# SkylerGao/MC_NeRF

Measured on AMD Instinct MI355X. Metric: train rays/sec (coarse+fine, 64+128 samples), higher is better.
Workload: dtype f16x3h; 1 GPU; Ball_Lego-shaped 110-view 800x800, coarse 4x128 @64 + fine 8x256 @128-grid, GLOBAL_OPTIM stage, fwd+bwd+allreduce+RAdam; precision=f16x3h, parallelism=dp1

## Files before the change

### mc_nerf_amd/build.py

```python
import os
import subprocess
import sys
from concurrent.futures import ThreadPoolExecutor

HERE = os.path.dirname(os.path.abspath(__file__))
CSRC = os.path.join(HERE, "csrc")
OUT = os.path.join(HERE, "libmcnerf.so")
SOURCES = ["api.hip", "pack.hip", "mlp_fwd.hip", "mlp_bwd.hip", "mlp_dw.hip", "pack16.hip", "mlp16_fwd.hip", "mlp16_bwd.hip", "mlp16_dw.hip", "mlp_x3_fwd.hip", "mlp_x3_bwd.hip", "mlp_x3_dw.hip", "composite.hip", "sample_pdf.hip", "select.hip", "rays.hip", "voxel.hip", "optim.hip", "optim_rows.hip", "camera.hip", "color_calib.hip", "errmap.hip", "lens.hip"]
HEADERS = ["mcnerf_common.h", "mcnerf_kernels.h", "mcnerf_wave.h", "mcnerf_16.h", "mcnerf_x3.h", "mcnerf_launch.h", "mcnerf_voxel.h", "mcnerf_multicam.h", "mcnerf_colorcal.h", "mcnerf_errmap.h", "mcnerf_maxkey.h", "mcnerf_compact.h", "mcnerf_hash.h", "mcnerf_rays.h", "mcnerf_lens.h", "mcnerf_optim_rows.h", os.path.join("..", "..", "include", "mcnerf.h")]
FILE_FLAGS = {s: ["-mllvm", "-pragma-unroll-threshold=200000", "-mllvm", "-amdgpu-mfma-vgpr-form"] for s in ("mlp_x3_fwd.hip", "mlp_x3_bwd.hip")}
FLAGS = ["--offload-arch=gfx950", "-O3", "-std=c++17", "-fPIC", "-munsafe-fp-atomics", "-ffp-contract=off", "-fno-slp-vectorize", "-Wall", "-Wno-unused-function"]


def _newer(a, b):
    return (not os.path.exists(b)) or os.path.getmtime(a) > os.path.getmtime(b)


def build(force=False, verbose=True):
    hipcc = os.environ.get("HIPCC", "/opt/rocm/bin/hipcc")
    objdir = os.path.join(HERE, "build")
    os.makedirs(objdir, exist_ok=True)
    hdrs = [os.path.normpath(os.path.join(CSRC, h)) for h in HEADERS]
    jobs = []
    for s in SOURCES:
        src, obj = os.path.join(CSRC, s), os.path.join(objdir, s.replace(".hip", ".o"))
        if force or _newer(src, obj) or any(_newer(h, obj) for h in hdrs):
            jobs.append((src, obj))

    def cc(job):
        src, obj = job
        cmd = [hipcc] + FLAGS + FILE_FLAGS.get(os.path.basename(src), []) + ["-c", src, "-o", obj]
        r = subprocess.run(cmd, capture_output=True, text=True)
        return src, r.returncode, r.stdout + r.stderr

    with ThreadPoolExecutor(max_workers=min(4, max(1, len(jobs)))) as ex:
        for src, rc, log in ex.map(cc, jobs):
            if verbose and log.strip():
                print(log)
            if rc != 0:
                raise RuntimeError(f"hipcc failed on {src}\n{log}")
            if verbose:
                print(f"[mc_nerf_amd.build] compiled {os.path.basename(src)}")
    objs = [os.path.join(objdir, s.replace(".hip", ".o")) for s in SOURCES]
    if jobs or not os.path.exists(OUT):
        cmd = [hipcc, "--offload-arch=gfx950", "-shared", "-fPIC", "-o", OUT] + objs
        r = subprocess.run(cmd, capture_output=True, text=True)
        if r.returncode != 0:
            raise RuntimeError("link failed\n" + r.stdout + r.stderr)
        if verbose:
            print(f"[mc_nerf_amd.build] linked {OUT}")
    return OUT


if __name__ == "__main__":
    build(force="--force" in sys.argv)
```

### mc_nerf_amd/csrc/mcnerf_x3.h

```cpp
#pragma once
#include "mcnerf_16.h"

#define MCNX3_SW 256.0f
#define MCNX3_SX 8.0f
#define MCNX3_SLABF 8
#define MCNX3_PF 2

#define MCNX3_WIDE_MIN 128
static inline constexpr int mcnx3_waves(int width) { return width >= MCNX3_WIDE_MIN ? 4 : 8; }

static inline int mcnx3_pad(int frags) { return (frags + MCNX3_SLABF - 1) / MCNX3_SLABF * MCNX3_SLABF; }
static inline Mcn16Stream mcnx3_repad(Mcn16Stream st) {
    int total = 0;
    for (int s = 0; s < st.nseg; ++s) {
        st.seg[s].first_frag = total;
        total += mcnx3_pad(st.seg[s].tiles * (st.seg[s].a.ksteps + st.seg[s].b.ksteps));
    }
    st.total_frags = total;
    return st;
}
static inline Mcn16Stream mcnx3_fwd_stream(const McnLayout& L) { return mcnx3_repad(mcn16_fwd_stream(L)); }
static inline Mcn16Stream mcnx3_bwd_stream(const McnLayout& L) { return mcnx3_repad(mcn16_bwd_stream(L)); }

static inline size_t mcnx3_slot_bytes(long long capacity, int width) { return 2 * mcn16_slot_bytes(capacity, width); }
static inline size_t mcnx3_enc_bytes(long long capacity) { return 2 * mcn16_enc_bytes(capacity); }
static inline size_t mcnx3_sh_bytes(long long capacity) { return (size_t)mcn16_cap_tiles(capacity) * 4096; }
static inline size_t mcnx3_dsh_bytes(long long capacity) { return 2 * mcn16_dsh_bytes(capacity); }

hipError_t mcnx3_launch_fwd(const Mcn16FwdArgs& a, hipStream_t st);
hipError_t mcnx3_launch_bwd(const Mcn16BwdArgs& a, hipStream_t st);
hipError_t mcnx3_launch_dw(const Mcn16DwArgs& a, hipStream_t st);
hipError_t mcnx3_launch_pack(const McnLayout& L, const float* params, void* packed_fwd, void* packed_bwd, unsigned* range_flags, hipStream_t st);

#ifdef __HIPCC__
typedef float f32x2_t __attribute__((ext_vector_type(2)));

__device__ __forceinline__ void mcnx3_split2(float a, float b, unsigned& hi, unsigned& lo) {
    const f16x2_t h = __builtin_convertvector((f32x2_t){a, b}, f16x2_t);
    const f32x2_t back = __builtin_convertvector(h, f32x2_t);
    const f16x2_t l = __builtin_convertvector((f32x2_t){a - back[0], b - back[1]}, f16x2_t);
    hi = __builtin_bit_cast(unsigned, h);
    lo = __builtin_bit_cast(unsigned, l);
}
__device__ __forceinline__ float mcnx3_val(unsigned hi, unsigned lo, int e) {
    const f16x2_t h = __builtin_bit_cast(f16x2_t, hi), l = __builtin_bit_cast(f16x2_t, lo);
    return (float)h[e] + (float)l[e];
}
template <int HI>
__device__ __forceinline__ float mcnx3_residual(float v, unsigned hw) {
    float r;
    if (HI) asm("v_fma_mix_f32 %0, %1, -1.0, %2 op_sel:[1,0,0] op_sel_hi:[1,0,0]" : "=v"(r) : "v"(hw), "v"(v));
    else asm("v_fma_mix_f32 %0, %1, -1.0, %2 op_sel_hi:[1,0,0]" : "=v"(r) : "v"(hw), "v"(v));
    return r;
}
__device__ __forceinline__ float mcnx3_relu(float x) {
    const int i = __builtin_bit_cast(int, x);
    return __builtin_bit_cast(float, i > 0 ? i : 0);
}
__device__ __forceinline__ f32x16 mcnx3_mfma(const u32x4_t& a, const u32x4_t& b, const f32x16& c) {
    return __builtin_amdgcn_mfma_f32_32x32x16_f16(__builtin_bit_cast(f16x8_t, a), __builtin_bit_cast(f16x8_t, b), c, 0, 0, 0);
}
__device__ __forceinline__ void mcnx3_mfma3(f32x16& acc, const u32x4_t& ah, const u32x4_t& al, const u32x4_t& bh, const u32x4_t& bl) {
    acc = mcnx3_mfma(al, bh, acc);
    acc = mcnx3_mfma(ah, bl, acc);
    acc = mcnx3_mfma(ah, bh, acc);
}

__device__ __forceinline__ void mcnx3_dma16(const char* ubase, unsigned voff, unsigned lds_dst) {
    unsigned keep;
    asm volatile("s_mov_b32 %0, m0\n\ts_mov_b32 m0, %3\n\ts_nop 0\n\tglobal_load_lds_dwordx4 %1, %2\n\ts_mov_b32 m0, %0"
                 : "=&s"(keep) : "v"(voff), "s"(ubase), "s"(lds_dst) : "memory");
}
template <int PPW>
__device__ __forceinline__ void mcnx3_ring_issue(Mcn16Ring& r) {
    const char* s = r.ubase + (size_t)r.src_slab * (MCN16_SLAB * 1024);
    const unsigned d = r.lds_base + r.issue_slot * (MCN16_SLAB * 1024) + r.lds_piece;
#pragma unroll
    for (int i = 0; i < PPW; ++i) mcnx3_dma16(s + i * 1024, r.voff, d + i * 1024);
    r.src_slab = (r.src_slab + 1 == r.n_slabs) ? 0 : r.src_slab + 1;
    r.issue_slot = (r.issue_slot + 1) & (MCN16_RING - 1);
}
template <int PPW>
__device__ __forceinline__ void mcnx3_ring_sync(Mcn16Ring& r) {
    asm volatile("s_waitcnt vmcnt(%0)\n\ts_barrier" ::"n"(PPW * (MCN16_AHEAD - 1)) : "memory");
    r.next_off = r.sync_slot * (MCN16_SLAB * 1024);
    r.sync_slot = (r.sync_slot + 1) & (MCN16_RING - 1);
    mcnx3_ring_issue<PPW>(r);
}
template <int PPW>
__device__ __forceinline__ void mcnx3_ring_start(Mcn16Ring& r, char* ring_lds, const void* packed, int n_slabs, int wave, int lane) {
    r.ubase = reinterpret_cast<const char*>(packed) + (PPW * wave) * 1024;
    r.voff = lane * 16;
    r.src = nullptr;
    r.lds_piece = (PPW * wave) * 1024;
    r.lds_base = (unsigned)reinterpret_cast<size_t>((mcn16_lds_ptr_t)ring_lds);
    r.src_slab = 0; r.n_slabs = n_slabs; r.issue_slot = 0; r.sync_slot = 0; r.next_off = 0;
#pragma unroll
    for (int i = 0; i < MCN16_AHEAD; ++i) mcnx3_ring_issue<PPW>(r);
    mcnx3_ring_sync<PPW>(r);
}
template <int F>
__host__ __device__ constexpr int mcnx3_sync_at(int q) {
    return (MCNX3_SLABF * q + MCNX3_SLABF - MCNX3_PF) < (F - 1) ? (MCNX3_SLABF * q + MCNX3_SLABF - MCNX3_PF) : (F - 1);
}
template <int F, int PPW>
__device__ __forceinline__ void mcnx3_before_mfma(Mcn16Ring& r, Mcn16Cursor& c, int f) {
    if ((f & (MCNX3_SLABF - 1)) == 0) c.cur = r.next_off;
    if (f == mcnx3_sync_at<F>(f / MCNX3_SLABF)) mcnx3_ring_sync<PPW>(r);
}
#define MCNX3_DMA_STEP 2
template <int PPW>
__device__ __forceinline__ void mcnx3_ring_piece(Mcn16Ring& r, int i) {
    switch (i) {
        case 0: asm volatile("global_load_lds_dwordx4 %0, %1" ::"v"(r.voff), "s"(r.piece_base) : "memory"); break;
        case 1: asm volatile("global_load_lds_dwordx4 %0, %1 offset:1024" ::"v"(r.voff), "s"(r.piece_base) : "memory"); break;
        case 2: asm volatile("global_load_lds_dwordx4 %0, %1 offset:2048" ::"v"(r.voff), "s"(r.piece_base) : "memory"); break;
        default: asm volatile("global_load_lds_dwordx4 %0, %1 offset:3072" ::"v"(r.voff), "s"(r.piece_base) : "memory"); break;
    }
}
template <int F, int PPW>
__device__ __forceinline__ void mcnx3_before_mfma_spread(Mcn16Ring& r, Mcn16Cursor& c, int f) {
    static_assert(PPW <= 4, "immediate offsets of the refill pieces");
    if ((f & (MCNX3_SLABF - 1)) == 0) c.cur = r.next_off;
    if (f == mcnx3_sync_at<F>(f / MCNX3_SLABF)) {
        asm volatile("s_waitcnt vmcnt(%0)\n\ts_barrier" ::"n"(PPW * (MCN16_AHEAD - 1)) : "memory");
        r.next_off = r.sync_slot * (MCN16_SLAB * 1024);
        r.sync_slot = (r.sync_slot + 1) & (MCN16_RING - 1);
        r.piece_base = r.ubase + (size_t)r.src_slab * (MCN16_SLAB * 1024);
        asm volatile("s_mov_b32 m0, %0" ::"s"(r.lds_base + r.issue_slot * (MCN16_SLAB * 1024) + r.lds_piece) : "memory");
        r.src_slab = (r.src_slab + 1 == r.n_slabs) ? 0 : r.src_slab + 1;
        r.issue_slot = (r.issue_slot + 1) & (MCN16_RING - 1);
    }
}
template <int F, int PPW>
__device__ __forceinline__ void mcnx3_gap_dma(Mcn16Ring& r, int gap) {
    constexpr int NQ = (F + MCNX3_SLABF - 1) / MCNX3_SLABF;
#pragma unroll
    for (int q = 0; q < NQ; ++q)
#pragma unroll
        for (int i = 0; i < PPW; ++i)
            if (gap == 3 * mcnx3_sync_at<F>(q) + 1 + MCNX3_DMA_STEP * i) mcnx3_ring_piece<PPW>(r, i);
}
template <int F, int PPW>
__device__ __forceinline__ void mcnx3_layer_end(Mcn16Ring& r) {
    constexpr int NQ = (F + MCNX3_SLABF - 1) / MCNX3_SLABF;
#pragma unroll
    for (int q = 0; q < NQ; ++q)
#pragma unroll
        for (int i = 0; i < PPW; ++i)
            if (3 * mcnx3_sync_at<F>(q) + 1 + MCNX3_DMA_STEP * i >= 3 * F) mcnx3_ring_piece<PPW>(r, i);
}
__device__ __forceinline__ unsigned mcnx3_frag_off(const Mcn16Ring& r, const Mcn16Cursor& c, int f_now, int f) {
    const bool next = (f / MCNX3_SLABF) != (f_now / MCNX3_SLABF);
    return (next ? r.next_off : c.cur) + (f & (MCNX3_SLABF - 1)) * 2048;
}

__device__ __forceinline__ void mcnx3_encode_values(const float (&p)[3], const float (&bw)[MCN_NFREQ], float (&E)[64]) {
    E[0] = p[0]; E[1] = p[1]; E[2] = p[2]; E[63] = 0.f;
#pragma unroll
    for (int a = 0; a < 3; ++a) {
        float S[MCN_NFREQ], C[MCN_NFREQ];
        mcn_sincos_octaves<MCN_NFREQ>(p[a], S, C);
#pragma unroll
        for (int f = 0; f < MCN_NFREQ; ++f) {
            E[3 + 20 * a + f] = S[f] * bw[f];
            E[3 + 20 * a + 10 + f] = C[f] * bw[f];
        }
    }
}
#endif
```

### mc_nerf_amd/csrc/mlp_x3_bwd.hip

```cpp
#include "mcnerf_x3.h"
#include "mcnerf_launch.h"

#define MCNX3_BWD_PREF_MINW 256
#include <cstdlib>

template <int W>
struct BwdX3Smem {
    static constexpr int WAVES = mcnx3_waves(W);
    static constexpr int oW2 = MCN16_RING * MCN16_SLAB * 1024;
    static constexpr int oBarf = oW2 + W * 4;
    static constexpr int MW = W >= 64 ? W / 64 : 1;
    static constexpr int oMask = oBarf + 16 * 4;
    static constexpr int oIdx = oMask + WAVES * 3 * MW * 256;
    static constexpr int oIn = oIdx + WAVES * 256;
    static constexpr int total = oIn + (W >= 256 ? WAVES * 16 * 256 : 0);
};

template <int W, int KSTEPS, int NTILES, int MODE, int PPW, bool HI>
__device__ __forceinline__ void mcnx3_bwd_seg(Mcn16Ring& ring, char* smem, int lane,
                                              const u32x4_t (&inh)[W / 16], const u32x4_t (&inl)[W / 16],
                                              u32x4_t (&outh)[W / 16], u32x4_t (&outl)[W / 16],
                                              const unsigned (&mk)[W >= 64 ? W / 64 : 1], f32x16 (&acc2)[2], char* save_lane) {
    constexpr int KS = W / 16, F = NTILES * KSTEPS, G = 3 * KSTEPS;
    constexpr bool EPI = MODE != 3;
    constexpr int NIT = EPI ? (MODE == 0 ? 16 : 20) : 0;
    constexpr int START = (G >= NIT + 8) ? 3 : 0;
    constexpr int IPG = EPI ? (NIT + (G - START) - 1) / (G - START) : 1;
    constexpr int LASTA = EPI ? START + 14 / IPG : 0;
    constexpr int SBASE = START + 16, SSTR = (G - SBASE) / 4 > 0 ? (G - SBASE) / 4 : 1;
    constexpr bool STAG = (MODE == 1 || MODE == 2) && IPG == 1 && (G - SBASE) / 4 >= 2;
    constexpr int NITG = STAG ? 16 : NIT;
    constexpr int INIT_G = (G - 8) > LASTA ? (G - 8) : LASTA;
    constexpr int INIT_N = (INIT_G + 3 <= G - 1) ? 4 : 1;
    Mcn16Cursor cur;
    u32x4_t afh[MCNX3_PF], afl[MCNX3_PF];
    f32x16 acc[2];
    float v0 = 0.f, v1 = 0.f;
    unsigned wkeep = 0u;
    auto acc_init = [&](f32x16& a, int t, int q) {
        if (MODE == 2) {
            const f16x8_t h8 = __builtin_bit_cast(f16x8_t, outh[2 * t + (q >> 1)]), l8 = __builtin_bit_cast(f16x8_t, outl[2 * t + (q >> 1)]);
#pragma unroll
            for (int e = 0; e < 4; ++e) a[4 * q + e] = ((float)h8[4 * (q & 1) + e] + (float)l8[4 * (q & 1) + e]) * MCNX3_SW;
        } else {
#pragma unroll
            for (int e = 0; e < 4; ++e) a[4 * q + e] = 0.f;
        }
    };
    auto item = [&](const f32x16& a, int t, int i) {
        if (i < 16) {
            const int p = i >> 1;
            const unsigned bits = MODE != 0 ? ((mk[t >> 1] >> (8 * (t & 1) + 7 - p)) & 0x00010001u) : 0u;
            if ((i & 1) == 0) {
                v0 = a[2 * p] * (1.0f / MCNX3_SW);
                v1 = a[2 * p + 1] * (1.0f / MCNX3_SW);
                const unsigned w = Mcn16T<false>::pack(v0, v1);
                wkeep = w;
                outh[2 * t + (p >> 2)][p & 3] = MODE != 0 ? mcn16_pkmul(w, bits) : w;
            } else {
                const unsigned w = Mcn16T<false>::pack(mcnx3_residual<0>(v0, wkeep), mcnx3_residual<1>(v1, wkeep));
                outl[2 * t + (p >> 2)][p & 3] = MODE != 0 ? mcn16_pkmul(w, bits) : w;
            }
        } else {
            const int k = i - 16, s = 2 * t + (k & 1);
            if (k < 2) mcn16_ws_store(outh[s], reinterpret_cast<u32x4_t*>(save_lane + s * 1024));
            else if (!HI) mcn16_ws_store(outl[s], reinterpret_cast<u32x4_t*>(save_lane + (KS + s) * 1024));
        }
    };
    cur.cur = ring.next_off;
#pragma unroll
    for (int i = 0; i < MCNX3_PF; ++i)
        if (i < F) {
            afh[i] = *reinterpret_cast<const u32x4_t*>(smem + ring.next_off + i * 2048 + lane * 16);
            afl[i] = *reinterpret_cast<const u32x4_t*>(smem + ring.next_off + i * 2048 + 1024 + lane * 16);
        }
    if (EPI) {
#pragma unroll
        for (int q = 0; q < 4; ++q) acc_init(acc[0], 0, q);
    }
#pragma unroll
    for (int t = 0; t < NTILES; ++t) {
#pragma unroll
        for (int s = 0; s < KSTEPS; ++s) {
            const int f = t * KSTEPS + s;
            mcnx3_before_mfma_spread<F, PPW>(ring, cur, f);
            const u32x4_t a_h = afh[f % MCNX3_PF], a_l = afl[f % MCNX3_PF];
            if (f + MCNX3_PF < F) {
                const unsigned o = mcnx3_frag_off(ring, cur, f, f + MCNX3_PF) + lane * 16;
                afh[f % MCNX3_PF] = *reinterpret_cast<const u32x4_t*>(smem + o);
                afl[f % MCNX3_PF] = *reinterpret_cast<const u32x4_t*>(smem + o + 1024);
            }
#pragma unroll
            for (int g = 0; g < 3; ++g) {
                const int gap = 3 * s + g;
                if (EPI && t > 0 && gap >= START) {
#pragma unroll
                    for (int i = (gap - START) * IPG; i < (gap - START + 1) * IPG; ++i)
                        if (i < NITG) item(acc[(t - 1) & 1], t - 1, i);
                    if (STAG && gap >= SBASE && (gap - SBASE) / SSTR < 4 && (gap - SBASE) % SSTR == 0)
                        item(acc[(t - 1) & 1], t - 1, 16 + (gap - SBASE) / SSTR);
                }
                if (EPI && t + 1 < NTILES && gap >= INIT_G && gap < INIT_G + INIT_N) {
#pragma unroll
                    for (int q = 0; q < 4; ++q)
                        if (INIT_N == 1 || q == gap - INIT_G) acc_init(acc[(t + 1) & 1], t + 1, q);
                }
                mcnx3_gap_dma<F, PPW>(ring, 3 * f + g);
                __builtin_amdgcn_sched_barrier(0);
                if (EPI) acc[t & 1] = mcnx3_mfma(g == 0 ? a_l : a_h, g == 1 ? inl[s] : inh[s], acc[t & 1]);
                else acc2[t & 1] = mcnx3_mfma(g == 0 ? a_l : a_h, g == 1 ? inl[s] : inh[s], acc2[t & 1]);
                __builtin_amdgcn_sched_barrier(0);
            }
        }
    }
    mcnx3_layer_end<F, PPW>(ring);
    if (EPI) {
#pragma unroll
        for (int i = 0; i < NIT; ++i) item(acc[(NTILES - 1) & 1], NTILES - 1, i);
    }
}

template <int W, bool HI>
__global__ __launch_bounds__(64 * mcnx3_waves(W), mcnx3_waves(W) / 4) void mlp_x3_bwd_kernel(Mcn16BwdArgs a) {
    using SM = BwdX3Smem<W>;
    constexpr int PL = HI ? 1 : 2;
    constexpr int WAVES = mcnx3_waves(W), ROWS = 32 * WAVES, PPW = 16 / WAVES;
    constexpr int NT = W / 32, KS = W / 16, MW = W >= 64 ? W / 64 : 1;
    extern __shared__ __attribute__((aligned(16))) char smem[];
    const int tid = threadIdx.x, lane = tid & 63, wave = __builtin_amdgcn_readfirstlane(tid >> 6);
    const int m = lane & 31, h = lane >> 5;
    const int D = a.lay.depth, skip = a.lay.skip;
    const long long total = a.count ? (long long)min(*a.count, a.max_rows) : (long long)a.n_rays * a.S;
    if ((long long)blockIdx.x * ROWS >= total) return;

    float* sw2 = reinterpret_cast<float*>(smem + SM::oW2);
    for (int i = tid; i < W; i += 64 * WAVES) sw2[i] = a.params[a.lay.pWs2 + i];
    float* sbarf = reinterpret_cast<float*>(smem + SM::oBarf);
    if (tid < MCN_NFREQ) sbarf[tid] = a.barf_w[tid];
    const float gmax = __uint_as_float(*a.gmax_bits);
    const float sg = mcn16_grad_scale(gmax);
    const float inv_sg = 1.0f / sg;
    __syncthreads();

    struct In { int ray; float zg, jit; f32x4 o, go; float dx, dy, dz, ox, oy, oz; };
    auto gather = [&](int ray, int j) -> In {
        In r;
        r.ray = ray;
        r.zg = a.zgrid[ray * a.z_stride + j];
        r.jit = a.jitter ? a.jitter[ray] : 0.f;
        const size_t addr = (size_t)ray * a.S + j;
        r.o = *reinterpret_cast<const f32x4*>(a.out + addr * 4);
        r.go = *reinterpret_cast<const f32x4*>(a.d_out + addr * 4);
        r.dx = a.rays_d[ray * 3]; r.dy = a.rays_d[ray * 3 + 1]; r.dz = a.rays_d[ray * 3 + 2];
        r.ox = a.rays_o[ray * 3]; r.oy = a.rays_o[ray * 3 + 1]; r.oz = a.rays_o[ray * 3 + 2];
        return r;
    };
    auto row_of = [&](long long pass_) -> long long {
        const long long g_ = (pass_ * WAVES + wave) * 32 + m;
        return g_ < total ? g_ : total - 1;
    };
    constexpr bool PREFB = W >= MCNX3_BWD_PREF_MINW;
    constexpr int SLABS_FULL = (W / 32) * (W / 16) / MCNX3_SLABF;
    constexpr int SLABS_ENC = (2 * (W / 16) + MCNX3_SLABF - 1) / MCNX3_SLABF;
    constexpr int N_IDX = PPW * (2 * SLABS_FULL - 1) < 63 ? PPW * (2 * SLABS_FULL - 1) : 63;
    constexpr int N_TOP = PPW * (SLABS_FULL + SLABS_ENC - 1) < 63 ? PPW * (SLABS_FULL + SLABS_ENC - 1) : 63;
    const unsigned in_lds = (unsigned)reinterpret_cast<size_t>((mcn16_lds_ptr_t)smem) + SM::oIn + wave * (16 * 256);
    const float* in_rd = reinterpret_cast<const float*>(smem + SM::oIn + wave * (16 * 256)) + lane;
    auto gather_dma = [&](int ray, int j) {
        mcn16_dma4(a.zgrid + ray * a.z_stride + j, in_lds);
        if (a.jitter) mcn16_dma4(a.jitter + ray, in_lds + 256);
        const size_t addr = ((size_t)ray * a.S + j) * 4;
#pragma unroll
        for (int c = 0; c < 4; ++c) {
            mcn16_dma4(a.out + addr + c, in_lds + (2 + c) * 256);
            mcn16_dma4(a.d_out + addr + c, in_lds + (6 + c) * 256);
        }
#pragma unroll
        for (int c = 0; c < 3; ++c) {
            mcn16_dma4(a.rays_d + ray * 3 + c, in_lds + (10 + c) * 256);
            mcn16_dma4(a.rays_o + ray * 3 + c, in_lds + (13 + c) * 256);
        }
    };
    auto read_in = [&](int ray) -> In {
        In r;
        r.ray = ray;
        r.zg = in_rd[0];
        r.jit = a.jitter ? in_rd[64] : 0.f;
        r.o = f32x4{in_rd[2 * 64], in_rd[3 * 64], in_rd[4 * 64], in_rd[5 * 64]};
        r.go = f32x4{in_rd[6 * 64], in_rd[7 * 64], in_rd[8 * 64], in_rd[9 * 64]};
        r.dx = in_rd[10 * 64]; r.dy = in_rd[11 * 64]; r.dz = in_rd[12 * 64];
        r.ox = in_rd[13 * 64]; r.oy = in_rd[14 * 64]; r.oz = in_rd[15 * 64];
        return r;
    };
    In cur;
    int ray_n = 0;
    {
        const long long gc0 = row_of(blockIdx.x);
        int ray0, j0;
        if (a.idx) { const int2 rj = a.idx[gc0]; ray0 = rj.x; j0 = rj.y; }
        else { ray0 = (int)(gc0 / a.S); j0 = (int)(gc0 - (long long)ray0 * a.S); }
        if (PREFB) { gather_dma(ray0, j0); ray_n = ray0; }
        else cur = gather(ray0, j0);
    }

    Mcn16Ring ring;
    mcnx3_ring_start<PPW>(ring, smem, a.packed, a.stream_slabs, wave, lane);
    const float* w2_h = sw2 + 4 * h;
    const unsigned idx_lds = (unsigned)reinterpret_cast<size_t>((mcn16_lds_ptr_t)smem) + SM::oIdx + wave * 256;

    constexpr bool MASK_DMA = W >= MCNX3_BWD_PREF_MINW;
    const unsigned mlds = ring.lds_base + SM::oMask + wave * (3 * MW * 256);
    auto mask_issue = [&](const unsigned* mask_lane, int slot, int buf) {
        if (MASK_DMA) {
#pragma unroll
            for (int i = 0; i < MW; ++i) mcn16_dma4(mask_lane + (size_t)slot * a.mask_slot_words + i, mlds + (buf * MW + i) * 256);
        }
    };
    auto mask_read = [&](const unsigned* mask_lane, unsigned (&mk)[MW], int buf, int slot) {
#pragma unroll
        for (int i = 0; i < MW; ++i) {
            if (MASK_DMA) mk[i] = *reinterpret_cast<const unsigned*>(smem + SM::oMask + wave * (3 * MW * 256) + (buf * MW + i) * 256 + lane * 4);
            else mk[i] = mask_lane[(size_t)slot * a.mask_slot_words + i];
        }
    };
    auto buf_of = [&](int slot) { return (D + 1 - slot) % 3; };
    auto mask_lane_of = [&](long long pass_) { return a.mask_ws + ((size_t)(pass_ * WAVES + wave) * 64 + lane) * MW; };
    unsigned mk0_s[MW], mk0_c[MW], mk0_t[MW];
    {
        const unsigned* ml0 = mask_lane_of(blockIdx.x);
        mask_issue(ml0, D, 0); mask_issue(ml0, D + 1, 1); mask_issue(ml0, D - 1, 2);
        if (!MASK_DMA) { mask_read(ml0, mk0_s, 0, D); mask_read(ml0, mk0_c, 1, D + 1); mask_read(ml0, mk0_t, 2, D - 1); }
        asm volatile("s_waitcnt vmcnt(0)" ::: "memory");
    }

    for (long long pass = blockIdx.x; pass * ROWS < total; pass += gridDim.x) {
        const long long tile = pass * WAVES + wave;
        const long long g = tile * 32 + m;
        const bool valid = g < total;
        const unsigned* mask_lane = mask_lane_of(pass);
        char* dy_lane = reinterpret_cast<char*>(a.dy_ws) + (size_t)tile * (PL * KS) * 1024 + lane * 16;
        if (PREFB) {
            asm volatile("s_waitcnt vmcnt(%0)" ::"n"(N_TOP) : "memory");
            cur = read_in(ray_n);
        }
        const int ray = cur.ray;
        unsigned mk_s[MW], mk_c[MW], mk_t[MW];
        float zv = cur.zg;
        if (a.jitter) zv = __fadd_rn(zv, cur.jit);
        const f32x4 o = cur.o;
        f32x4 go = cur.go;
        if (!valid) go = f32x4{0.f, 0.f, 0.f, 0.f};
        const float x = cur.dx, y = cur.dy, z = cur.dz;
        float p[3];
        p[0] = __fadd_rn(cur.ox, __fmul_rn(x, zv));
        p[1] = __fadd_rn(cur.oy, __fmul_rn(y, zv));
        p[2] = __fadd_rn(cur.oz, __fmul_rn(z, zv));
        float bas[9];
        mcn_sh_basis(x, y, z, bas);
        float dpre[3];
#pragma unroll
        for (int c = 0; c < 3; ++c) dpre[c] = go[1 + c] * o[1 + c] * (1.f - o[1 + c]) * sg;
        const float dsg = go[0] * sg;
        u32x4_t dshh[2], dshl[2];
#pragma unroll
        for (int s = 0; s < 2; ++s)
#pragma unroll
            for (int d = 0; d < 4; ++d) {
                float v[2];
#pragma unroll
                for (int u = 0; u < 2; ++u) {
                    const int n0 = mcn16_chan(s, 0, 2 * d + u), n1 = n0 + 4;
                    const float va = n0 < MCN_NSH ? dpre[n0 / 9] * bas[n0 % 9] : (n0 == MCN_NSH ? dsg : 0.f);
                    const float vb = n1 < MCN_NSH ? dpre[n1 / 9] * bas[n1 % 9] : (n1 == MCN_NSH ? dsg : 0.f);
                    v[u] = h ? vb : va;
                }
                unsigned wh, wl;
                mcnx3_split2(v[0], v[1], wh, wl);
                dshh[s][d] = wh; dshl[s][d] = wl;
            }
        {
            char* e = reinterpret_cast<char*>(a.dsh_ws) + (size_t)tile * (PL * 2) * 1024 + lane * 16;
            mcn16_ws_store(dshh[0], reinterpret_cast<u32x4_t*>(e));
            mcn16_ws_store(dshh[1], reinterpret_cast<u32x4_t*>(e + 1024));
            if (!HI) {
                mcn16_ws_store(dshl[0], reinterpret_cast<u32x4_t*>(e + 2048));
                mcn16_ws_store(dshl[1], reinterpret_cast<u32x4_t*>(e + 3072));
            }
        }

        if (MASK_DMA) mask_read(mask_lane, mk_s, 0, D);
        else {
#pragma unroll
            for (int i = 0; i < MW; ++i) { mk_s[i] = mk0_s[i]; mk_c[i] = mk0_c[i]; mk_t[i] = mk0_t[i]; }
        }
        const long long pass_n = pass + gridDim.x;
        if (a.idx) {
            const long long gn = (pass_n * WAVES + wave) * 32 + (lane >> 1);
            mcn16_dma4(reinterpret_cast<const int*>(a.idx) + 2 * (gn < total ? gn : total - 1) + (lane & 1), idx_lds);
        }
        const bool want_rays = a.d_rays_o || a.d_rays_d;
        f32x4 shs[4];
#pragma unroll
        for (int q = 0; q < 4; ++q) shs[q] = f32x4{0.f, 0.f, 0.f, 0.f};
        if (PREFB && want_rays) {
#pragma unroll
            for (int q = 0; q < 4; ++q)
                shs[q] = *reinterpret_cast<const f32x4*>(reinterpret_cast<const char*>(a.sh_ws) + (size_t)tile * 4096 + q * 1024 + lane * 16);
        }
        u32x4_t xah[KS], xal[KS], xbh[KS], xbl[KS];
        f32x16 denc[2];
#pragma unroll
        for (int t = 0; t < 2; ++t)
#pragma unroll
            for (int e = 0; e < 16; ++e) denc[t][e] = 0.f;
#pragma unroll
        for (int s = 0; s < KS; ++s) {
            const f32x4 wa = *reinterpret_cast<const f32x4*>(w2_h + 16 * s), wb = *reinterpret_cast<const f32x4*>(w2_h + 16 * s + 8);
            const int t = s >> 1;
#pragma unroll
            for (int d = 0; d < 4; ++d) {
                const float va = (d < 2 ? wa[2 * d] : wb[2 * d - 4]) * dsg, vb = (d < 2 ? wa[2 * d + 1] : wb[2 * d - 3]) * dsg;
                const int i = 4 * (s & 1) + d;
                const unsigned bits = (mk_s[t >> 1] >> (8 * (t & 1) + 7 - i)) & 0x00010001u;
                unsigned wh, wl;
                mcnx3_split2(va, vb, wh, wl);
                xah[s][d] = mcn16_pkmul(wh, bits);
                xal[s][d] = mcn16_pkmul(wl, bits);
            }
            mcn16_ws_store(xah[s], reinterpret_cast<u32x4_t*>(dy_lane + (size_t)D * a.slot_bytes + s * 1024));
            if (!HI) mcn16_ws_store(xal[s], reinterpret_cast<u32x4_t*>(dy_lane + (size_t)D * a.slot_bytes + (KS + s) * 1024));
        }
        if (D >= 2) mask_issue(mask_lane, D - 2, buf_of(D - 2));
        unsigned mpend[MW];
        if (!MASK_DMA && D >= 2) mask_read(mask_lane, mpend, 0, D - 2);
        mcnx3_bwd_seg<W, KS, NT, 0, PPW, HI>(ring, smem, lane, xah, xal, xbh, xbl, mk_s, denc, nullptr);
        if (MASK_DMA) mask_read(mask_lane, mk_c, 1, D + 1);
        {
            u32x4_t dih[KS], dil[KS];
            dih[0] = dshh[0]; dih[1] = dshh[1]; dil[0] = dshl[0]; dil[1] = dshl[1];
            mcnx3_bwd_seg<W, 2, NT, 1, PPW, HI>(ring, smem, lane, dih, dil, xah, xal, mk_c, denc, dy_lane + (size_t)(D + 1) * a.slot_bytes);
        }
        if (D >= 3) mask_issue(mask_lane, D - 3, buf_of(D - 3));
        if (MASK_DMA) mask_read(mask_lane, mk_t, 2, D - 1);
        mcnx3_bwd_seg<W, KS, NT, 2, PPW, HI>(ring, smem, lane, xah, xal, xbh, xbl, mk_t, denc, dy_lane + (size_t)(D - 1) * a.slot_bytes);
        auto trunk_masks = [&](int l) {
            if (MASK_DMA) {
                if (l >= 3) mask_issue(mask_lane, l - 3, buf_of(l - 3));
                mask_read(mask_lane, mk_t, buf_of(l - 1), l - 1);
            } else {
#pragma unroll
                for (int i = 0; i < MW; ++i) mk_t[i] = mpend[i];
                if (l >= 2) mask_read(mask_lane, mpend, 0, l - 2);
            }
            if (l == 1 && pass_n * ROWS < total) {
                const unsigned* mln = mask_lane_of(pass_n);
                mask_issue(mln, D, 0); mask_issue(mln, D + 1, 1); mask_issue(mln, D - 1, 2);
                if (!MASK_DMA) { mask_read(mln, mk0_s, 0, D); mask_read(mln, mk0_c, 1, D + 1); mask_read(mln, mk0_t, 2, D - 1); }
            }
        };
        auto next_rows = [&]() {
            asm volatile("s_waitcnt vmcnt(%0)" ::"n"(N_IDX) : "memory");
            int rn, jn;
            if (a.idx) {
                const int2 rj = *reinterpret_cast<const int2*>(smem + SM::oIdx + wave * 256 + m * 8);
                rn = rj.x; jn = rj.y;
            } else {
                const long long gn = row_of(pass_n);
                rn = (int)(gn / a.S); jn = (int)(gn - (long long)rn * a.S);
            }
            gather_dma(rn, jn);
            ray_n = rn;
        };
        for (int l = D - 1; l >= 1; l -= 2) {
            if (PREFB && l == 1) next_rows();
            trunk_masks(l);
            if (l == skip) mcnx3_bwd_seg<W, KS, 2, 3, PPW, HI>(ring, smem, lane, xbh, xbl, xah, xal, mk_t, denc, nullptr);
            mcnx3_bwd_seg<W, KS, NT, 1, PPW, HI>(ring, smem, lane, xbh, xbl, xah, xal, mk_t, denc, dy_lane + (size_t)(l - 1) * a.slot_bytes);
            if (l - 1 >= 1) {
                if (PREFB && l - 1 == 1) next_rows();
                trunk_masks(l - 1);
                if (l - 1 == skip) mcnx3_bwd_seg<W, KS, 2, 3, PPW, HI>(ring, smem, lane, xah, xal, xbh, xbl, mk_t, denc, nullptr);
                mcnx3_bwd_seg<W, KS, NT, 1, PPW, HI>(ring, smem, lane, xah, xal, xbh, xbl, mk_t, denc, dy_lane + (size_t)(l - 2) * a.slot_bytes);
            } else {
#pragma unroll
                for (int s = 0; s < KS; ++s) { xbh[s] = xah[s]; xbl[s] = xal[s]; }
            }
        }
        In nxt = cur;
        if (PREFB && D < 2) {
            next_rows();
        }
        if (!PREFB) {
            int rn, jn;
            if (a.idx) {
                const int2 rj = *reinterpret_cast<const int2*>(smem + SM::oIdx + wave * 256 + m * 8);
                rn = rj.x; jn = rj.y;
            } else {
                const long long gn = row_of(pass_n);
                rn = (int)(gn / a.S); jn = (int)(gn - (long long)rn * a.S);
            }
            nxt = gather(rn, jn);
        }
        if (!PREFB && want_rays) {
#pragma unroll
            for (int q = 0; q < 4; ++q)
                shs[q] = *reinterpret_cast<const f32x4*>(reinterpret_cast<const char*>(a.sh_ws) + (size_t)tile * 4096 + q * 1024 + lane * 16);
        }
        mcnx3_bwd_seg<W, KS, 2, 3, PPW, HI>(ring, smem, lane, xbh, xbl, xah, xal, mk_t, denc, nullptr);
        auto settle = [&]() {
            if (PREFB && D >= 2) return;
            asm volatile("s_waitcnt vmcnt(0)" ::: "memory");
            asm volatile("" : "+v"(nxt.ray), "+v"(nxt.zg), "+v"(nxt.jit), "+v"(nxt.o), "+v"(nxt.go));
            asm volatile("" : "+v"(nxt.dx), "+v"(nxt.dy), "+v"(nxt.dz), "+v"(nxt.ox), "+v"(nxt.oy), "+v"(nxt.oz));
            if (!MASK_DMA) {
#pragma unroll
                for (int i = 0; i < MW; ++i) asm volatile("" : "+v"(mk0_s[i]), "+v"(mk0_c[i]), "+v"(mk0_t[i]));
            }
        };

        if (want_rays) {
            auto dch = [&](int ch) -> float {
                const int hh = (ch >> 2) & 1;
                const float v = denc[ch >> 5][4 * ((ch >> 3) & 3) + (ch & 3)];
                return (h == hh) ? v : 0.f;
            };
            float dpos[3];
#pragma unroll
            for (int ax = 0; ax < 3; ++ax) {
                float acc = dch(ax);
                float S[MCN_NFREQ], C[MCN_NFREQ];
                mcn_sincos_octaves<MCN_NFREQ>(p[ax], S, C);
#pragma unroll
                for (int f = 0; f < MCN_NFREQ; ++f) {
                    const float k = (float)(1 << f) * sbarf[f];
                    acc = fmaf(k * C[f], dch(3 + 20 * ax + f), acc);
                    acc = fmaf(-k * S[f], dch(3 + 20 * ax + 10 + f), acc);
                }
                dpos[ax] = acc * (1.0f / MCNX3_SW);
            }
            float ddir[3] = {0.f, 0.f, 0.f};
            {
                const float C1 = 0.4886025119029199f, C20 = 1.0925484305920792f, C22 = 0.31539156525252005f, C24 = 0.5462742152960396f;
                const float gx[9] = {0.f, 0.f, 0.f, -C1, C20 * y, 0.f, -2.f * C22 * x, -C20 * z, 2.f * C24 * x};
                const float gy[9] = {0.f, -C1, 0.f, 0.f, C20 * x, -C20 * z, -2.f * C22 * y, 0.f, -2.f * C24 * y};
                const float gz[9] = {0.f, 0.f, C1, 0.f, 0.f, -C20 * y, 4.f * C22 * z, -C20 * x, 0.f};
#pragma unroll
                for (int r = 0; r < 16; ++r) {
                    const float v = shs[r >> 2][r & 3];
                    const int n0 = 8 * (r >> 2) + (r & 3), n1 = n0 + 4;
                    const float kx = h ? (n1 < MCN_NSH ? dpre[n1 / 9] * gx[n1 % 9] : 0.f) : (n0 < MCN_NSH ? dpre[n0 / 9] * gx[n0 % 9] : 0.f);
                    const float ky = h ? (n1 < MCN_NSH ? dpre[n1 / 9] * gy[n1 % 9] : 0.f) : (n0 < MCN_NSH ? dpre[n0 / 9] * gy[n0 % 9] : 0.f);
                    const float kz = h ? (n1 < MCN_NSH ? dpre[n1 / 9] * gz[n1 % 9] : 0.f) : (n0 < MCN_NSH ? dpre[n0 / 9] * gz[n0 % 9] : 0.f);
                    ddir[0] = fmaf(kx, v, ddir[0]); ddir[1] = fmaf(ky, v, ddir[1]); ddir[2] = fmaf(kz, v, ddir[2]);
                }
            }
            float red[6];
#pragma unroll
            for (int c = 0; c < 3; ++c) {
                const float dp = dpos[c] + __shfl_xor(dpos[c], 32);
                const float dd = ddir[c] + __shfl_xor(ddir[c], 32);
                red[c] = dp * inv_sg;
                red[3 + c] = (dp * zv + dd) * inv_sg;
            }
            settle();
            const int rkey = valid ? ray : -1;
            const int rprev = __shfl_up(rkey, 1, 32);
            int head = (m == 0 || rprev != rkey) ? 1 : 0;
#pragma unroll
            for (int off = 1; off < 32; off <<= 1) {
                const int hup = __shfl_up(head, off, 32);
                const bool take = (m >= off) && !head;
#pragma unroll
                for (int c = 0; c < 6; ++c) {
                    const float up = __shfl_up(red[c], off, 32);
                    red[c] += take ? up : 0.f;
                }
                if (m >= off) head |= hup;
            }
            const int rnext = __shfl_down(rkey, 1, 32);
            if (h == 0 && valid && (m == 31 || rnext != rkey)) {
#pragma unroll
                for (int c = 0; c < 3; ++c) {
                    if (a.d_rays_o) atomicAdd(a.d_rays_o + ray * 3 + c, red[c]);
                    if (a.d_rays_d) atomicAdd(a.d_rays_d + ray * 3 + c, red[3 + c]);
                }
            }
        }
        if (!want_rays) settle();
        if (!PREFB) cur = nxt;
    }
    asm volatile("s_waitcnt vmcnt(0)" ::: "memory");
}

hipError_t mcnx3_launch_bwd(const Mcn16BwdArgs& a, hipStream_t st) {
    return mcn_for_width(a.lay.width, [&](auto w) {
        constexpr int W = decltype(w)::value, WAVES = mcnx3_waves(W);
        void (*kern)(Mcn16BwdArgs) = mcn16_hi_planes_only(a.dtype) ? mlp_x3_bwd_kernel<W, true> : mlp_x3_bwd_kernel<W, false>;
        return mcn_launch(kern, mcn_persistent_grid(mcn_passes(mcn_max_rows(a), 32 * WAVES)), 64 * WAVES, BwdX3Smem<W>::total, st, a);
    });
}
```

### mc_nerf_amd/csrc/mlp_x3_fwd.hip

```cpp
#include "mcnerf_x3.h"
#include "mcnerf_launch.h"

template <int W>
struct FwdX3Smem {
    static constexpr int oBias = MCN16_RING * MCN16_SLAB * 1024;
    static constexpr int oW2 = oBias + (MCN_MAXD + 2) * W * 4;
    static constexpr int oBc2 = oW2 + W * 4;
    static constexpr int oIdx = oBc2 + 32 * 4;
    static constexpr int oIn = oIdx + mcnx3_waves(W) * 256;
    static constexpr int total = oIn + mcnx3_waves(W) * 8 * 256;
};

template <int W, int SV, int KENC, int KHID, int EPI, int PPW>
__device__ __forceinline__ void mcnx3_layer(Mcn16Ring& ring, char* smem, int lane,
                                            const u32x4_t (&ench)[MCN16_ENCKS], const u32x4_t (&encl)[MCN16_ENCKS],
                                            const u32x4_t (&inh)[W / 16], const u32x4_t (&inl)[W / 16],
                                            u32x4_t (&outh)[W / 16], u32x4_t (&outl)[W / 16], const float* bias_h,
                                            const float* w2_h, float& dot, char* save_lane, unsigned* mask_lane) {
    constexpr bool SAVE = SV != 0, HI = SV == 2;
    constexpr int NT = W / 32, KS = W / 16, KTOT = KENC + KHID, F = NT * KTOT, MW = W >= 64 ? W / 64 : 1;
    constexpr int G = 3 * KTOT;
    constexpr bool HAS2 = SAVE || EPI == 1;
    constexpr int IPW = HAS2 ? 3 : 2;
    constexpr int NST = SAVE ? (HI ? 2 : 4) : 0;
    constexpr int NIT = 8 * IPW + NST;
    constexpr int NWI = 8 * IPW;
    constexpr int ROOM = G - 3 - 2 * NST;
    constexpr int IPGA = ROOM > 0 ? (NWI + ROOM - 1) / ROOM : 99;
    constexpr bool STAG = SAVE && IPGA <= 2;
    constexpr int START = STAG ? 3 : (G >= NIT + 4 ? 3 : 0);
    constexpr int IPG = STAG ? IPGA : (NIT + (G - START) - 1) / (G - START);
    constexpr int NITG = STAG ? NWI : NIT;
    constexpr int LASTG = START + (NITG + IPG - 1) / IPG - 1;
    constexpr int SBASE = LASTG + 1, SSTR = STAG ? (G - SBASE) / NST : 1;
    constexpr int BIAS_G = (G - 6) > LASTG ? (G - 6) : LASTG;
    Mcn16Cursor cur;
    unsigned mw[MW];
#pragma unroll
    for (int i = 0; i < MW; ++i) mw[i] = 0u;
    u32x4_t afh[MCNX3_PF], afl[MCNX3_PF];
    f32x16 acc[2];
    unsigned mb = 0u;
    float v0 = 0.f, v1 = 0.f;
    unsigned wkeep = 0u;
    auto bias_init = [&](f32x16& a, int t) {
#pragma unroll
        for (int q = 0; q < 4; ++q) {
            const f32x4 b = *reinterpret_cast<const f32x4*>(bias_h + 32 * t + 8 * q);
#pragma unroll
            for (int e = 0; e < 4; ++e) a[4 * q + e] = b[e];
        }
    };
    auto item = [&](const f32x16& a, int t, int i) {
        if (i < 8 * IPW) {
            const int p = i / IPW, ph = i % IPW;
            if (ph == 0) {
                v0 = mcnx3_relu(a[2 * p] * (1.0f / MCNX3_SW));
                v1 = mcnx3_relu(a[2 * p + 1] * (1.0f / MCNX3_SW));
                const unsigned w = Mcn16T<false>::pack(v0, v1);
                wkeep = w;
                outh[2 * t + (p >> 2)][p & 3] = w;
            } else if (ph == IPW - 1) {
                outl[2 * t + (p >> 2)][p & 3] = Mcn16T<false>::pack(mcnx3_residual<0>(v0, wkeep), mcnx3_residual<1>(v1, wkeep));
            } else {
                if (SAVE) {
                    mb = (p == 0) ? mcn16_nz(wkeep) : ((mb << 1) | mcn16_nz(wkeep));
                    if (p == 7) mw[t >> 1] |= mb << (8 * (t & 1));
                }
                if (EPI == 1) {
                    const f32x2_t ww = *reinterpret_cast<const f32x2_t*>(w2_h + 32 * t + 8 * (p >> 1) + 2 * (p & 1));
                    dot = fmaf(v0, ww[0], dot);
                    dot = fmaf(v1, ww[1], dot);
                }
            }
        } else if (SAVE) {
            const int k = i - 8 * IPW;
            const int s = 2 * t + (k & 1);
            if (k < 2) mcn16_ws_store(outh[s], reinterpret_cast<u32x4_t*>(save_lane + s * 1024));
            else mcn16_ws_store(outl[s], reinterpret_cast<u32x4_t*>(save_lane + (KS + s) * 1024));
        }
    };
    cur.cur = ring.next_off;
#pragma unroll
    for (int i = 0; i < MCNX3_PF; ++i)
        if (i < F) {
            afh[i] = *reinterpret_cast<const u32x4_t*>(smem + ring.next_off + i * 2048 + lane * 16);
            afl[i] = *reinterpret_cast<const u32x4_t*>(smem + ring.next_off + i * 2048 + 1024 + lane * 16);
        }
    bias_init(acc[0], 0);
#pragma unroll
    for (int t = 0; t < NT; ++t) {
#pragma unroll
        for (int s = 0; s < KTOT; ++s) {
            const int f = t * KTOT + s;
            mcnx3_before_mfma_spread<F, PPW>(ring, cur, f);
            const u32x4_t a_h = afh[f % MCNX3_PF], a_l = afl[f % MCNX3_PF];
            if (f + MCNX3_PF < F) {
                const unsigned o = mcnx3_frag_off(ring, cur, f, f + MCNX3_PF) + lane * 16;
                afh[f % MCNX3_PF] = *reinterpret_cast<const u32x4_t*>(smem + o);
                afl[f % MCNX3_PF] = *reinterpret_cast<const u32x4_t*>(smem + o + 1024);
            }
            const u32x4_t b_h = s < KENC ? ench[s < KENC ? s : 0] : inh[s >= KENC ? s - KENC : 0];
            const u32x4_t b_l = s < KENC ? encl[s < KENC ? s : 0] : inl[s >= KENC ? s - KENC : 0];
#pragma unroll
            for (int g = 0; g < 3; ++g) {
                const int gap = 3 * s + g;
                if (t > 0 && gap >= START) {
#pragma unroll
                    for (int i = (gap - START) * IPG; i < (gap - START + 1) * IPG; ++i)
                        if (i < NITG) item(acc[(t - 1) & 1], t - 1, i);
                    if (STAG && gap >= SBASE && (gap - SBASE) / SSTR < NST && (gap - SBASE) % SSTR == 0)
                        item(acc[(t - 1) & 1], t - 1, 8 * IPW + (gap - SBASE) / SSTR);
                }
                if (gap == BIAS_G && t + 1 < NT) bias_init(acc[(t + 1) & 1], t + 1);
                mcnx3_gap_dma<F, PPW>(ring, 3 * f + g);
                __builtin_amdgcn_sched_barrier(0);
                acc[t & 1] = mcnx3_mfma(g == 0 ? a_l : a_h, g == 1 ? b_l : b_h, acc[t & 1]);
                __builtin_amdgcn_sched_barrier(0);
            }
        }
    }
    mcnx3_layer_end<F, PPW>(ring);
#pragma unroll
    for (int i = 0; i < NIT; ++i) item(acc[(NT - 1) & 1], NT - 1, i);
    if (SAVE) {
#pragma unroll
        for (int i = 0; i < MW; ++i) mcn16_ws_store(mw[i], mask_lane + i);
    }
}


template <int W, int SV>
__global__ __launch_bounds__(64 * mcnx3_waves(W), mcnx3_waves(W) / 4) void mlp_x3_fwd_kernel(Mcn16FwdArgs a) {
    using SM = FwdX3Smem<W>;
    constexpr bool SAVE = SV != 0, HI = SV == 2;
    constexpr int PL = HI ? 1 : 2;
    constexpr int WAVES = mcnx3_waves(W), ROWS = 32 * WAVES, PPW = 16 / WAVES;
    constexpr int KS = W / 16, MW = W >= 64 ? W / 64 : 1;
    constexpr float SXW = MCNX3_SX * MCNX3_SW;
    extern __shared__ __attribute__((aligned(16))) char smem[];
    const int tid = threadIdx.x, lane = tid & 63, wave = __builtin_amdgcn_readfirstlane(tid >> 6);
    const int m = lane & 31, h = lane >> 5;
    const int D = a.lay.depth, skip = a.lay.skip;
    const long long total = a.count ? (long long)min(*a.count, a.max_rows) : (long long)a.n_rays * a.S;
    if ((long long)blockIdx.x * ROWS >= total) return;

    float* sbias = reinterpret_cast<float*>(smem + SM::oBias);
    float* sw2 = reinterpret_cast<float*>(smem + SM::oW2);
    float* sbc2 = reinterpret_cast<float*>(smem + SM::oBc2);
    for (int l = 0; l < D; ++l)
        for (int i = tid; i < W; i += 64 * WAVES) sbias[l * W + i] = a.params[a.lay.pB[l] + i] * SXW;
    for (int i = tid; i < W; i += 64 * WAVES) {
        sbias[D * W + i] = a.params[a.lay.pBs1 + i] * SXW;
        sbias[(D + 1) * W + i] = a.params[a.lay.pBc1 + i] * SXW;
        sw2[i] = a.params[a.lay.pWs2 + i];
    }
    if (tid < 32) {
        const int row = tid < MCN_NSH ? mcn_sh_row(tid, a.lay.sh_deg) : -1;
        sbc2[tid] = row >= 0 ? a.params[a.lay.pBc2 + row] * SXW : 0.f;
    }
    const float bs2 = a.params[a.lay.pBs2];
    float bw[MCN_NFREQ];
#pragma unroll
    for (int f = 0; f < MCN_NFREQ; ++f) bw[f] = a.barf_w[f];
    __syncthreads();

    constexpr bool PREF = WAVES == 4;
    constexpr int SLABS_FULL = (W / 32) * (W / 16) / MCNX3_SLABF, SLABS_L0 = ((W / 32) * MCN16_ENCKS + MCNX3_SLABF - 1) / MCNX3_SLABF;
    constexpr int SLABS_SH2 = (W / 16 + MCNX3_SLABF - 1) / MCNX3_SLABF;
    constexpr int N_IDX = PPW * (SLABS_L0 + SLABS_FULL - 1) < 63 ? PPW * (SLABS_L0 + SLABS_FULL - 1) : 63;
    constexpr int N_TOP = PPW * (SLABS_FULL + SLABS_SH2 - 1) < 63 ? PPW * (SLABS_FULL + SLABS_SH2 - 1) : 63;
    const unsigned idx_lds = (unsigned)reinterpret_cast<size_t>((mcn16_lds_ptr_t)smem) + SM::oIdx + wave * 256;
    const unsigned in_lds = (unsigned)reinterpret_cast<size_t>((mcn16_lds_ptr_t)smem) + SM::oIn + wave * (8 * 256);
    const float* in_rd = reinterpret_cast<const float*>(smem + SM::oIn + wave * (8 * 256)) + lane;
    auto row_of = [&](long long pass_) -> long long {
        const long long g_ = (pass_ * WAVES + wave) * 32 + m;
        return g_ < total ? g_ : total - 1;
    };
    auto gather_dma = [&](int ray_, int j_) {
        mcn16_dma4(a.zgrid + ray_ * a.z_stride + j_, in_lds);
        if (a.jitter) mcn16_dma4(a.jitter + ray_, in_lds + 256);
#pragma unroll
        for (int c = 0; c < 3; ++c) {
            mcn16_dma4(a.rays_d + ray_ * 3 + c, in_lds + (2 + c) * 256);
            mcn16_dma4(a.rays_o + ray_ * 3 + c, in_lds + (5 + c) * 256);
        }
    };
    int ray_n = 0, j_n = 0;
    {
        const long long gc0 = row_of(blockIdx.x);
        if (a.idx) { const int2 rj = a.idx[gc0]; ray_n = rj.x; j_n = rj.y; }
        else { ray_n = (int)(gc0 / a.S); j_n = (int)(gc0 - (long long)ray_n * a.S); }
        if (PREF) {
            gather_dma(ray_n, j_n);
            asm volatile("s_waitcnt vmcnt(0)" ::: "memory");
        }
    }

    Mcn16Ring ring;
    mcnx3_ring_start<PPW>(ring, smem, a.packed, a.stream_slabs, wave, lane);

    const float* bias_h = sbias + 4 * h;
    const float* w2_h = sw2 + 4 * h;

    for (long long pass = blockIdx.x; pass * ROWS < total; pass += gridDim.x) {
        const long long tile = pass * WAVES + wave;
        const long long g = tile * 32 + m;
        const bool valid = g < total;
        const long long gc = valid ? g : total - 1;
        const long long pass_n = pass + gridDim.x;
        int ray, j;
        float zv, dx, dy, dz, ox, oy, oz;
        if (PREF) {
            ray = ray_n; j = j_n;
            asm volatile("s_waitcnt vmcnt(%0)" ::"n"(N_TOP) : "memory");
            zv = in_rd[0];
            if (a.jitter) zv = __fadd_rn(zv, in_rd[64]);
            dx = in_rd[2 * 64]; dy = in_rd[3 * 64]; dz = in_rd[4 * 64];
            ox = in_rd[5 * 64]; oy = in_rd[6 * 64]; oz = in_rd[7 * 64];
        } else {
            if (a.idx) { const int2 rj = a.idx[gc]; ray = rj.x; j = rj.y; }
            else { ray = (int)(gc / a.S); j = (int)(gc - (long long)ray * a.S); }
            zv = a.zgrid[ray * a.z_stride + j];
            if (a.jitter) zv = __fadd_rn(zv, a.jitter[ray]);
            dx = a.rays_d[ray * 3 + 0]; dy = a.rays_d[ray * 3 + 1]; dz = a.rays_d[ray * 3 + 2];
            ox = a.rays_o[ray * 3 + 0]; oy = a.rays_o[ray * 3 + 1]; oz = a.rays_o[ray * 3 + 2];
        }
        float p[3];
        p[0] = __fadd_rn(ox, __fmul_rn(dx, zv));
        p[1] = __fadd_rn(oy, __fmul_rn(dy, zv));
        p[2] = __fadd_rn(oz, __fmul_rn(dz, zv));
        if (PREF && a.idx) {
            const long long gn = (pass_n * WAVES + wave) * 32 + (lane >> 1);
            mcn16_dma4(reinterpret_cast<const int*>(a.idx) + 2 * (gn < total ? gn : total - 1) + (lane & 1), idx_lds);
        }
        const int addr = ray * a.S + j;
        u32x4_t ench[MCN16_ENCKS], encl[MCN16_ENCKS];
        {
            float E[64];
            mcnx3_encode_values(p, bw, E);
#pragma unroll
            for (int s = 0; s < MCN16_ENCKS; ++s)
#pragma unroll
                for (int d = 0; d < 4; ++d) {
                    const int c0 = mcn16_chan(s, 0, 2 * d), c1 = mcn16_chan(s, 0, 2 * d + 1);
                    unsigned wh, wl;
                    mcnx3_split2((h ? E[c0 + 4] : E[c0]) * MCNX3_SX, (h ? E[c1 + 4] : E[c1]) * MCNX3_SX, wh, wl);
                    ench[s][d] = wh; encl[s][d] = wl;
                }
        }
        char* act_lane = SAVE ? reinterpret_cast<char*>(a.act_ws) + (size_t)tile * (PL * KS) * 1024 + lane * 16 : nullptr;
        unsigned* mask_lane = SAVE ? a.mask_ws + ((size_t)tile * 64 + lane) * MW : nullptr;
        if (SAVE) {
            char* e = reinterpret_cast<char*>(a.enc_ws) + (size_t)tile * (PL * MCN16_ENCKS) * 1024 + lane * 16;
#pragma unroll
            for (int s = 0; s < MCN16_ENCKS; ++s) {
                mcn16_ws_store(ench[s], reinterpret_cast<u32x4_t*>(e + s * 1024));
                if (!HI) mcn16_ws_store(encl[s], reinterpret_cast<u32x4_t*>(e + (MCN16_ENCKS + s) * 1024));
            }
        }

        u32x4_t xah[KS], xal[KS], xbh[KS], xbl[KS];
        float dot = 0.f;
        mcnx3_layer<W, SV, MCN16_ENCKS, 0, 0, PPW>(ring, smem, lane, ench, encl, xah, xal, xbh, xbl, bias_h, nullptr, dot, act_lane, mask_lane);
        for (int l = 1; l < D; l += 2) {
            char* sl = SAVE ? act_lane + (size_t)l * a.slot_bytes : nullptr;
            unsigned* ml = SAVE ? mask_lane + (size_t)l * a.mask_slot_words : nullptr;
            if (l == skip) mcnx3_layer<W, SV, MCN16_ENCKS, KS, 0, PPW>(ring, smem, lane, ench, encl, xbh, xbl, xah, xal, bias_h + l * W, nullptr, dot, sl, ml);
            else mcnx3_layer<W, SV, 0, KS, 0, PPW>(ring, smem, lane, ench, encl, xbh, xbl, xah, xal, bias_h + l * W, nullptr, dot, sl, ml);
            if (l + 1 < D) {
                sl = SAVE ? act_lane + (size_t)(l + 1) * a.slot_bytes : nullptr;
                ml = SAVE ? mask_lane + (size_t)(l + 1) * a.mask_slot_words : nullptr;
                if (l + 1 == skip) mcnx3_layer<W, SV, MCN16_ENCKS, KS, 0, PPW>(ring, smem, lane, ench, encl, xah, xal, xbh, xbl, bias_h + (l + 1) * W, nullptr, dot, sl, ml);
                else mcnx3_layer<W, SV, 0, KS, 0, PPW>(ring, smem, lane, ench, encl, xah, xal, xbh, xbl, bias_h + (l + 1) * W, nullptr, dot, sl, ml);
            } else {
#pragma unroll
                for (int s = 0; s < KS; ++s) { xbh[s] = xah[s]; xbl[s] = xal[s]; }
            }
        }
        mcnx3_layer<W, SV, 0, KS, 1, PPW>(ring, smem, lane, ench, encl, xbh, xbl, xah, xal, bias_h + D * W, w2_h, dot,
                                            SAVE ? act_lane + (size_t)D * a.slot_bytes : nullptr, SAVE ? mask_lane + (size_t)D * a.mask_slot_words : nullptr);
        if (PREF) {
            asm volatile("s_waitcnt vmcnt(%0)" ::"n"(N_IDX) : "memory");
            if (a.idx) {
                const int2 rj = *reinterpret_cast<const int2*>(smem + SM::oIdx + wave * 256 + m * 8);
                ray_n = rj.x; j_n = rj.y;
            } else {
                const long long gn = row_of(pass_n);
                ray_n = (int)(gn / a.S); j_n = (int)(gn - (long long)ray_n * a.S);
            }
            gather_dma(ray_n, j_n);
        }
        mcnx3_layer<W, SV, 0, KS, 0, PPW>(ring, smem, lane, ench, encl, xbh, xbl, xah, xal, bias_h + (D + 1) * W, nullptr, dot,
                                            SAVE ? act_lane + (size_t)(D + 1) * a.slot_bytes : nullptr, SAVE ? mask_lane + (size_t)(D + 1) * a.mask_slot_words : nullptr);
        f32x16 acc;
#pragma unroll
        for (int q = 0; q < 4; ++q) {
            const f32x4 b = *reinterpret_cast<const f32x4*>(sbc2 + 8 * q + 4 * h);
#pragma unroll
            for (int e = 0; e < 4; ++e) acc[4 * q + e] = b[e];
        }
        {
            Mcn16Cursor cur;
#pragma unroll
            for (int s = 0; s < KS; ++s) {
                mcnx3_before_mfma<KS, PPW>(ring, cur, s);
                const unsigned o = cur.cur + (s & (MCNX3_SLABF - 1)) * 2048 + lane * 16;
                const u32x4_t a_h = *reinterpret_cast<const u32x4_t*>(smem + o);
                const u32x4_t a_l = *reinterpret_cast<const u32x4_t*>(smem + o + 1024);
                mcnx3_mfma3(acc, a_h, a_l, xah[s], xal[s]);
            }
        }
#pragma unroll
        for (int e = 0; e < 16; ++e) acc[e] *= 1.0f / SXW;
        if (SAVE) {
            char* e = reinterpret_cast<char*>(a.sh_ws) + (size_t)tile * 4096 + lane * 16;
#pragma unroll
            for (int q = 0; q < 4; ++q)
                mcn16_ws_store(f32x4{acc[4 * q], acc[4 * q + 1], acc[4 * q + 2], acc[4 * q + 3]}, reinterpret_cast<f32x4*>(e + q * 1024));
        }
        float bas[9];
        mcn_sh_basis(dx, dy, dz, bas);
        float pre[3] = {0.f, 0.f, 0.f};
#pragma unroll
        for (int r = 0; r < 16; ++r) {
            const int n0 = 8 * (r >> 2) + (r & 3), n1 = n0 + 4;
            const float b0 = n0 < MCN_NSH ? bas[n0 % 9] : 0.f, b1 = n1 < MCN_NSH ? bas[n1 % 9] : 0.f;
            const float contrib = acc[r] * (h ? b1 : b0);
            const int c0 = n0 / 9, c1 = n1 / 9;
#pragma unroll
            for (int c = 0; c < 3; ++c) {
                const bool in0 = n0 < MCN_NSH && c0 == c, in1 = n1 < MCN_NSH && c1 == c;
                if (in0 && in1) pre[c] += contrib;
                else if (in0) pre[c] += h ? 0.f : contrib;
                else if (in1) pre[c] += h ? contrib : 0.f;
            }
        }
        const float sigma = (dot + __shfl_xor(dot, 32)) * (1.0f / MCNX3_SX) + bs2;
        f32x4 o;
        o[0] = sigma;
#pragma unroll
        for (int c = 0; c < 3; ++c) {
            const float pc = pre[c] + __shfl_xor(pre[c], 32);
            o[1 + c] = 1.0f / (1.0f + expf(-pc));
        }
        if (valid && h == 0) *reinterpret_cast<f32x4*>(a.out + (size_t)addr * 4) = o;
    }
    asm volatile("s_waitcnt vmcnt(0)" ::: "memory");
}

hipError_t mcnx3_launch_fwd(const Mcn16FwdArgs& a, hipStream_t st) {
    return mcn_for_width(a.lay.width, [&](auto w) {
        constexpr int W = decltype(w)::value, WAVES = mcnx3_waves(W);
        void (*kern)(Mcn16FwdArgs) = !a.act_ws ? mlp_x3_fwd_kernel<W, 0> : mcn16_hi_planes_only(a.dtype) ? mlp_x3_fwd_kernel<W, 2> : mlp_x3_fwd_kernel<W, 1>;
        return mcn_launch(kern, mcn_persistent_grid(mcn_passes(mcn_max_rows(a), 32 * WAVES)), 64 * WAVES, FwdX3Smem<W>::total, st, a);
    });
}
```

Baseline: 1.092 million rays/s.

## Add 8-wave variant of x3 MLP fwd/bwd kernels for width 128

Adds an alternate kernel instantiation for width-128 x3 MLP forward and backward that uses 8 waves per block instead of 4. It uses prefetch depth 1, drops the LDS mask staging and reloads lane-dependent addresses through an opaque value to keep register pressure low. Tail tiles are remapped so duplicate 'twin' tiles redo the last live work. The intent is more waves in flight to hide LDS and MFMA latency. The cost is extra address recomputation and shuffles via ds_bpermute, and an environment override can pick the wave count.

```diff
diff --git a/mc_nerf_amd/build.py b/mc_nerf_amd/build.py
--- a/mc_nerf_amd/build.py
+++ b/mc_nerf_amd/build.py
@@ -7,7 +7,7 @@
 CSRC = os.path.join(HERE, "csrc")
 OUT = os.path.join(HERE, "libmcnerf.so")
 SOURCES = ["api.hip", "pack.hip", "mlp_fwd.hip", "mlp_bwd.hip", "mlp_dw.hip", "pack16.hip", "mlp16_fwd.hip", "mlp16_bwd.hip", "mlp16_dw.hip", "mlp_x3_fwd.hip", "mlp_x3_bwd.hip", "mlp_x3_dw.hip", "composite.hip", "sample_pdf.hip", "select.hip", "rays.hip", "voxel.hip", "optim.hip", "optim_rows.hip", "camera.hip", "color_calib.hip", "errmap.hip", "lens.hip"]
-HEADERS = ["mcnerf_common.h", "mcnerf_kernels.h", "mcnerf_wave.h", "mcnerf_16.h", "mcnerf_x3.h", "mcnerf_launch.h", "mcnerf_voxel.h", "mcnerf_multicam.h", "mcnerf_colorcal.h", "mcnerf_errmap.h", "mcnerf_maxkey.h", "mcnerf_compact.h", "mcnerf_hash.h", "mcnerf_rays.h", "mcnerf_lens.h", "mcnerf_optim_rows.h", os.path.join("..", "..", "include", "mcnerf.h")]
+HEADERS = ["mcnerf_common.h", "mcnerf_kernels.h", "mcnerf_wave.h", "mcnerf_16.h", "mcnerf_x3.h", "mcnerf_x3_waves.h", "mcnerf_launch.h", "mcnerf_voxel.h", "mcnerf_multicam.h", "mcnerf_colorcal.h", "mcnerf_errmap.h", "mcnerf_maxkey.h", "mcnerf_compact.h", "mcnerf_hash.h", "mcnerf_rays.h", "mcnerf_lens.h", "mcnerf_optim_rows.h", os.path.join("..", "..", "include", "mcnerf.h")]
 FILE_FLAGS = {s: ["-mllvm", "-pragma-unroll-threshold=200000", "-mllvm", "-amdgpu-mfma-vgpr-form"] for s in ("mlp_x3_fwd.hip", "mlp_x3_bwd.hip")}
 FLAGS = ["--offload-arch=gfx950", "-O3", "-std=c++17", "-fPIC", "-munsafe-fp-atomics", "-ffp-contract=off", "-fno-slp-vectorize", "-Wall", "-Wno-unused-function"]
 
diff --git a/mc_nerf_amd/csrc/mcnerf_x3.h b/mc_nerf_amd/csrc/mcnerf_x3.h
--- a/mc_nerf_amd/csrc/mcnerf_x3.h
+++ b/mc_nerf_amd/csrc/mcnerf_x3.h
@@ -8,6 +8,8 @@
 
 #define MCNX3_WIDE_MIN 128
 static inline constexpr int mcnx3_waves(int width) { return width >= MCNX3_WIDE_MIN ? 4 : 8; }
+static inline constexpr bool mcnx3_has_alt_waves(int width) { return width == 128; }
+static inline constexpr int mcnx3_alt_waves(int width) { return width == 128 ? 8 : mcnx3_waves(width); }
 
 static inline int mcnx3_pad(int frags) { return (frags + MCNX3_SLABF - 1) / MCNX3_SLABF * MCNX3_SLABF; }
 static inline Mcn16Stream mcnx3_repad(Mcn16Stream st) {
@@ -60,6 +62,11 @@
 __device__ __forceinline__ f32x16 mcnx3_mfma(const u32x4_t& a, const u32x4_t& b, const f32x16& c) {
     return __builtin_amdgcn_mfma_f32_32x32x16_f16(__builtin_bit_cast(f16x8_t, a), __builtin_bit_cast(f16x8_t, b), c, 0, 0, 0);
 }
+__device__ __forceinline__ int mcnx3_opaque(int v) { asm volatile("" : "+v"(v)); return v; }
+__device__ __forceinline__ float mcnx3_swap32(float x, int lane) {
+    return __builtin_bit_cast(float, __builtin_amdgcn_ds_bpermute((lane ^ 32) << 2, __builtin_bit_cast(int, x)));
+}
+
 __device__ __forceinline__ void mcnx3_mfma3(f32x16& acc, const u32x4_t& ah, const u32x4_t& al, const u32x4_t& bh, const u32x4_t& bl) {
     acc = mcnx3_mfma(al, bh, acc);
     acc = mcnx3_mfma(ah, bl, acc);
@@ -99,9 +106,9 @@
     for (int i = 0; i < MCN16_AHEAD; ++i) mcnx3_ring_issue<PPW>(r);
     mcnx3_ring_sync<PPW>(r);
 }
-template <int F>
+template <int F, int PF = MCNX3_PF>
 __host__ __device__ constexpr int mcnx3_sync_at(int q) {
-    return (MCNX3_SLABF * q + MCNX3_SLABF - MCNX3_PF) < (F - 1) ? (MCNX3_SLABF * q + MCNX3_SLABF - MCNX3_PF) : (F - 1);
+    return (MCNX3_SLABF * q + MCNX3_SLABF - PF) < (F - 1) ? (MCNX3_SLABF * q + MCNX3_SLABF - PF) : (F - 1);
 }
 template <int F, int PPW>
 __device__ __forceinline__ void mcnx3_before_mfma(Mcn16Ring& r, Mcn16Cursor& c, int f) {
@@ -118,11 +125,11 @@
         default: asm volatile("global_load_lds_dwordx4 %0, %1 offset:3072" ::"v"(r.voff), "s"(r.piece_base) : "memory"); break;
     }
 }
-template <int F, int PPW>
+template <int F, int PPW, int PF = MCNX3_PF>
 __device__ __forceinline__ void mcnx3_before_mfma_spread(Mcn16Ring& r, Mcn16Cursor& c, int f) {
     static_assert(PPW <= 4, "immediate offsets of the refill pieces");
     if ((f & (MCNX3_SLABF - 1)) == 0) c.cur = r.next_off;
-    if (f == mcnx3_sync_at<F>(f / MCNX3_SLABF)) {
+    if (f == mcnx3_sync_at<F, PF>(f / MCNX3_SLABF)) {
         asm volatile("s_waitcnt vmcnt(%0)\n\ts_barrier" ::"n"(PPW * (MCN16_AHEAD - 1)) : "memory");
         r.next_off = r.sync_slot * (MCN16_SLAB * 1024);
         r.sync_slot = (r.sync_slot + 1) & (MCN16_RING - 1);
@@ -132,23 +139,23 @@
         r.issue_slot = (r.issue_slot + 1) & (MCN16_RING - 1);
     }
 }
-template <int F, int PPW>
+template <int F, int PPW, int PF = MCNX3_PF>
 __device__ __forceinline__ void mcnx3_gap_dma(Mcn16Ring& r, int gap) {
     constexpr int NQ = (F + MCNX3_SLABF - 1) / MCNX3_SLABF;
 #pragma unroll
     for (int q = 0; q < NQ; ++q)
 #pragma unroll
         for (int i = 0; i < PPW; ++i)
-            if (gap == 3 * mcnx3_sync_at<F>(q) + 1 + MCNX3_DMA_STEP * i) mcnx3_ring_piece<PPW>(r, i);
+            if (gap == 3 * mcnx3_sync_at<F, PF>(q) + 1 + MCNX3_DMA_STEP * i) mcnx3_ring_piece<PPW>(r, i);
 }
-template <int F, int PPW>
+template <int F, int PPW, int PF = MCNX3_PF>
 __device__ __forceinline__ void mcnx3_layer_end(Mcn16Ring& r) {
     constexpr int NQ = (F + MCNX3_SLABF - 1) / MCNX3_SLABF;
 #pragma unroll
     for (int q = 0; q < NQ; ++q)
 #pragma unroll
         for (int i = 0; i < PPW; ++i)
-            if (3 * mcnx3_sync_at<F>(q) + 1 + MCNX3_DMA_STEP * i >= 3 * F) mcnx3_ring_piece<PPW>(r, i);
+            if (3 * mcnx3_sync_at<F, PF>(q) + 1 + MCNX3_DMA_STEP * i >= 3 * F) mcnx3_ring_piece<PPW>(r, i);
 }
 __device__ __forceinline__ unsigned mcnx3_frag_off(const Mcn16Ring& r, const Mcn16Cursor& c, int f_now, int f) {
     const bool next = (f / MCNX3_SLABF) != (f_now / MCNX3_SLABF);
diff --git a/mc_nerf_amd/csrc/mcnerf_x3_waves.h b/mc_nerf_amd/csrc/mcnerf_x3_waves.h
--- /dev/null
+++ b/mc_nerf_amd/csrc/mcnerf_x3_waves.h
@@ -0,0 +1,23 @@
+#pragma once
+#include <cstdlib>
+
+#pragma GCC visibility push(hidden)
+
+enum McnX3Chain { MCNX3_CHAIN_FWD_SAVE = 0, MCNX3_CHAIN_FWD_NOSAVE = 1, MCNX3_CHAIN_BWD = 2 };
+
+static constexpr int MCNX3_W128_WAVES[3] = {8, 8, 8};
+
+inline int mcnx3_w128_override() {
+    static const int v = [] {
+        const char* s = std::getenv("MCNERF_X3_WAVES128");
+        const int n = s ? std::atoi(s) : 0;
+        return (n == 4 || n == 8) ? n : 0;
+    }();
+    return v;
+}
+inline int mcnx3_w128_waves(McnX3Chain k) {
+    const int o = mcnx3_w128_override();
+    return o ? o : MCNX3_W128_WAVES[k];
+}
+
+#pragma GCC visibility pop
diff --git a/mc_nerf_amd/csrc/mlp_x3_bwd.hip b/mc_nerf_amd/csrc/mlp_x3_bwd.hip
--- a/mc_nerf_amd/csrc/mlp_x3_bwd.hip
+++ b/mc_nerf_amd/csrc/mlp_x3_bwd.hip
@@ -1,22 +1,24 @@
 #include "mcnerf_x3.h"
 #include "mcnerf_launch.h"
-
-#define MCNX3_BWD_PREF_MINW 256
+#include "mcnerf_x3_waves.h"
+
 #include <cstdlib>
 
-template <int W>
+template <int W, int WV = mcnx3_waves(W)>
 struct BwdX3Smem {
-    static constexpr int WAVES = mcnx3_waves(W);
+    static constexpr int WAVES = WV;
     static constexpr int oW2 = MCN16_RING * MCN16_SLAB * 1024;
     static constexpr int oBarf = oW2 + W * 4;
     static constexpr int MW = W >= 64 ? W / 64 : 1;
     static constexpr int oMask = oBarf + 16 * 4;
-    static constexpr int oIdx = oMask + WAVES * 3 * MW * 256;
+    static constexpr bool ALT = WV != mcnx3_waves(W);
+    static constexpr int oIdx = oMask + (ALT ? 0 : WAVES * 3 * MW * 256);
     static constexpr int oIn = oIdx + WAVES * 256;
-    static constexpr int total = oIn + (W >= 256 ? WAVES * 16 * 256 : 0);
+    static constexpr bool PREF = W >= 256;
+    static constexpr int total = oIn + (PREF ? WAVES * 16 * 256 : 0);
 };
 
-template <int W, int KSTEPS, int NTILES, int MODE, int PPW, bool HI>
+template <int W, int KSTEPS, int NTILES, int MODE, int PPW, bool HI, int PF = MCNX3_PF>
 __device__ __forceinline__ void mcnx3_bwd_seg(Mcn16Ring& ring, char* smem, int lane,
                                               const u32x4_t (&inh)[W / 16], const u32x4_t (&inl)[W / 16],
                                               u32x4_t (&outh)[W / 16], u32x4_t (&outl)[W / 16],
@@ -33,7 +35,7 @@
     constexpr int INIT_G = (G - 8) > LASTA ? (G - 8) : LASTA;
     constexpr int INIT_N = (INIT_G + 3 <= G - 1) ? 4 : 1;
     Mcn16Cursor cur;
-    u32x4_t afh[MCNX3_PF], afl[MCNX3_PF];
+    u32x4_t afh[PF], afl[PF];
     f32x16 acc[2];
     float v0 = 0.f, v1 = 0.f;
     unsigned wkeep = 0u;
@@ -69,7 +71,7 @@
     };
     cur.cur = ring.next_off;
 #pragma unroll
-    for (int i = 0; i < MCNX3_PF; ++i)
+    for (int i = 0; i < PF; ++i)
         if (i < F) {
             afh[i] = *reinterpret_cast<const u32x4_t*>(smem + ring.next_off + i * 2048 + lane * 16);
             afl[i] = *reinterpret_cast<const u32x4_t*>(smem + ring.next_off + i * 2048 + 1024 + lane * 16);
@@ -83,12 +85,12 @@
 #pragma unroll
         for (int s = 0; s < KSTEPS; ++s) {
             const int f = t * KSTEPS + s;
-            mcnx3_before_mfma_spread<F, PPW>(ring, cur, f);
-            const u32x4_t a_h = afh[f % MCNX3_PF], a_l = afl[f % MCNX3_PF];
-            if (f + MCNX3_PF < F) {
-                const unsigned o = mcnx3_frag_off(ring, cur, f, f + MCNX3_PF) + lane * 16;
-                afh[f % MCNX3_PF] = *reinterpret_cast<const u32x4_t*>(smem + o);
-                afl[f % MCNX3_PF] = *reinterpret_cast<const u32x4_t*>(smem + o + 1024);
+            mcnx3_before_mfma_spread<F, PPW, PF>(ring, cur, f);
+            const u32x4_t a_h = afh[f % PF], a_l = afl[f % PF];
+            if (f + PF < F) {
+                const unsigned o = mcnx3_frag_off(ring, cur, f, f + PF) + lane * 16;
+                afh[f % PF] = *reinterpret_cast<const u32x4_t*>(smem + o);
+                afl[f % PF] = *reinterpret_cast<const u32x4_t*>(smem + o + 1024);
             }
 #pragma unroll
             for (int g = 0; g < 3; ++g) {
@@ -105,7 +107,7 @@
                     for (int q = 0; q < 4; ++q)
                         if (INIT_N == 1 || q == gap - INIT_G) acc_init(acc[(t + 1) & 1], t + 1, q);
                 }
-                mcnx3_gap_dma<F, PPW>(ring, 3 * f + g);
+                mcnx3_gap_dma<F, PPW, PF>(ring, 3 * f + g);
                 __builtin_amdgcn_sched_barrier(0);
                 if (EPI) acc[t & 1] = mcnx3_mfma(g == 0 ? a_l : a_h, g == 1 ? inl[s] : inh[s], acc[t & 1]);
                 else acc2[t & 1] = mcnx3_mfma(g == 0 ? a_l : a_h, g == 1 ? inl[s] : inh[s], acc2[t & 1]);
@@ -113,19 +115,21 @@
             }
         }
     }
-    mcnx3_layer_end<F, PPW>(ring);
+    mcnx3_layer_end<F, PPW, PF>(ring);
     if (EPI) {
 #pragma unroll
         for (int i = 0; i < NIT; ++i) item(acc[(NTILES - 1) & 1], NTILES - 1, i);
     }
 }
 
-template <int W, bool HI>
-__global__ __launch_bounds__(64 * mcnx3_waves(W), mcnx3_waves(W) / 4) void mlp_x3_bwd_kernel(Mcn16BwdArgs a) {
-    using SM = BwdX3Smem<W>;
+template <int W, bool HI, int WV>
+__device__ __forceinline__ void mlp_x3_bwd_body(const Mcn16BwdArgs& a) {
+    using SM = BwdX3Smem<W, WV>;
     constexpr int PL = HI ? 1 : 2;
-    constexpr int WAVES = mcnx3_waves(W), ROWS = 32 * WAVES, PPW = 16 / WAVES;
+    constexpr int WAVES = WV, ROWS = 32 * WAVES, PPW = 16 / WAVES;
     constexpr int NT = W / 32, KS = W / 16, MW = W >= 64 ? W / 64 : 1;
+    constexpr bool ALT = SM::ALT;
+    constexpr int PF = ALT ? 1 : MCNX3_PF;
     extern __shared__ __attribute__((aligned(16))) char smem[];
     const int tid = threadIdx.x, lane = tid & 63, wave = __builtin_amdgcn_readfirstlane(tid >> 6);
     const int m = lane & 31, h = lane >> 5;
@@ -155,11 +159,17 @@
         r.ox = a.rays_o[ray * 3]; r.oy = a.rays_o[ray * 3 + 1]; r.oz = a.rays_o[ray * 3 + 2];
         return r;
     };
-    auto row_of = [&](long long pass_) -> long long {
-        const long long g_ = (pass_ * WAVES + wave) * 32 + m;
+    const long long live_tiles = (total + 127) / 128 * 4;
+    auto tile_of = [&](long long pass_) -> long long {
+        const long long t_ = pass_ * WAVES + wave;
+        return ALT && t_ >= live_tiles ? t_ - 4 : t_;
+    };
+    auto row_of = [&](long long pass_, int m_) -> long long {
+        const long long g_ = tile_of(pass_) * 32 + m_;
         return g_ < total ? g_ : total - 1;
     };
-    constexpr bool PREFB = W >= MCNX3_BWD_PREF_MINW;
+    constexpr bool PREFB = SM::PREF;
+    constexpr bool SHS_EARLY = W >= 256;
     constexpr int SLABS_FULL = (W / 32) * (W / 16) / MCNX3_SLABF;
     constexpr int SLABS_ENC = (2 * (W / 16) + MCNX3_SLABF - 1) / MCNX3_SLABF;
     constexpr int N_IDX = PPW * (2 * SLABS_FULL - 1) < 63 ? PPW * (2 * SLABS_FULL - 1) : 63;
@@ -195,7 +205,7 @@
     In cur;
     int ray_n = 0;
     {
-        const long long gc0 = row_of(blockIdx.x);
+        const long long gc0 = row_of(blockIdx.x, m);
         int ray0, j0;
         if (a.idx) { const int2 rj = a.idx[gc0]; ray0 = rj.x; j0 = rj.y; }
         else { ray0 = (int)(gc0 / a.S); j0 = (int)(gc0 - (long long)ray0 * a.S); }
@@ -208,7 +218,7 @@
     const float* w2_h = sw2 + 4 * h;
     const unsigned idx_lds = (unsigned)reinterpret_cast<size_t>((mcn16_lds_ptr_t)smem) + SM::oIdx + wave * 256;
 
-    constexpr bool MASK_DMA = W >= MCNX3_BWD_PREF_MINW;
+    constexpr bool MASK_DMA = SM::PREF;
     const unsigned mlds = ring.lds_base + SM::oMask + wave * (3 * MW * 256);
     auto mask_issue = [&](const unsigned* mask_lane, int slot, int buf) {
         if (MASK_DMA) {
@@ -229,16 +239,31 @@
     {
         const unsigned* ml0 = mask_lane_of(blockIdx.x);
         mask_issue(ml0, D, 0); mask_issue(ml0, D + 1, 1); mask_issue(ml0, D - 1, 2);
-        if (!MASK_DMA) { mask_read(ml0, mk0_s, 0, D); mask_read(ml0, mk0_c, 1, D + 1); mask_read(ml0, mk0_t, 2, D - 1); }
+        if (!MASK_DMA && !ALT) { mask_read(ml0, mk0_s, 0, D); mask_read(ml0, mk0_c, 1, D + 1); mask_read(ml0, mk0_t, 2, D - 1); }
         asm volatile("s_waitcnt vmcnt(0)" ::: "memory");
     }
 
+    const int lane0 = lane, m0 = m, h0 = h;
+    const float* w2_h0 = w2_h;
     for (long long pass = blockIdx.x; pass * ROWS < total; pass += gridDim.x) {
-        const long long tile = pass * WAVES + wave;
+        const int lane = ALT ? mcnx3_opaque(lane0) : lane0, m = ALT ? lane & 31 : m0, h = ALT ? lane >> 5 : h0;
+        const float* w2_h = ALT ? sw2 + 4 * h : w2_h0;
+        auto ln = [&]() { return ALT ? mcnx3_opaque(lane0) : lane; };
+        const long long tile = tile_of(pass);
+        const bool twin = ALT && pass * WAVES + wave >= live_tiles;
         const long long g = tile * 32 + m;
         const bool valid = g < total;
-        const unsigned* mask_lane = mask_lane_of(pass);
-        char* dy_lane = reinterpret_cast<char*>(a.dy_ws) + (size_t)tile * (PL * KS) * 1024 + lane * 16;
+        const unsigned* mask_lane = ALT ? nullptr : mask_lane_of(pass);
+        char* dy_lane0 = ALT ? nullptr : reinterpret_cast<char*>(a.dy_ws) + (size_t)tile * (PL * KS) * 1024 + lane * 16;
+        auto dy_of = [&](int l) -> char* {
+            if (ALT) return reinterpret_cast<char*>(a.dy_ws) + ((size_t)tile * (PL * KS) * 1024 + (size_t)l * a.slot_bytes) + ln() * 16;
+            return dy_lane0 + (size_t)l * a.slot_bytes;
+        };
+        auto mask_at = [&](unsigned (&mk)[MW], int slot) {
+            const unsigned* ml = a.mask_ws + ((size_t)tile * 64 * MW + (size_t)slot * a.mask_slot_words) + ln() * MW;
+#pragma unroll
+            for (int i = 0; i < MW; ++i) mk[i] = ml[i];
+        };
         if (PREFB) {
             asm volatile("s_waitcnt vmcnt(%0)" ::"n"(N_TOP) : "memory");
             cur = read_in(ray_n);
@@ -279,7 +304,7 @@
                 dshh[s][d] = wh; dshl[s][d] = wl;
             }
         {
-            char* e = reinterpret_cast<char*>(a.dsh_ws) + (size_t)tile * (PL * 2) * 1024 + lane * 16;
+            char* e = reinterpret_cast<char*>(a.dsh_ws) + (size_t)tile * (PL * 2) * 1024 + ln() * 16;
             mcn16_ws_store(dshh[0], reinterpret_cast<u32x4_t*>(e));
             mcn16_ws_store(dshh[1], reinterpret_cast<u32x4_t*>(e + 1024));
             if (!HI) {
@@ -289,23 +314,25 @@
         }
 
         if (MASK_DMA) mask_read(mask_lane, mk_s, 0, D);
+        else if (ALT) { mask_at(mk_s, D); mask_at(mk_c, D + 1); mask_at(mk_t, D - 1); }
         else {
 #pragma unroll
             for (int i = 0; i < MW; ++i) { mk_s[i] = mk0_s[i]; mk_c[i] = mk0_c[i]; mk_t[i] = mk0_t[i]; }
         }
         const long long pass_n = pass + gridDim.x;
         if (a.idx) {
-            const long long gn = (pass_n * WAVES + wave) * 32 + (lane >> 1);
-            mcn16_dma4(reinterpret_cast<const int*>(a.idx) + 2 * (gn < total ? gn : total - 1) + (lane & 1), idx_lds);
+            const int lane_i = ln();
+            const long long gn = tile_of(pass_n) * 32 + (lane_i >> 1);
+            mcn16_dma4(reinterpret_cast<const int*>(a.idx) + 2 * (gn < total ? gn : total - 1) + (lane_i & 1), idx_lds);
         }
         const bool want_rays = a.d_rays_o || a.d_rays_d;
         f32x4 shs[4];
 #pragma unroll
         for (int q = 0; q < 4; ++q) shs[q] = f32x4{0.f, 0.f, 0.f, 0.f};
-        if (PREFB && want_rays) {
+        if (SHS_EARLY && want_rays) {
 #pragma unroll
             for (int q = 0; q < 4; ++q)
-                shs[q] = *reinterpret_cast<const f32x4*>(reinterpret_cast<const char*>(a.sh_ws) + (size_t)tile * 4096 + q * 1024 + lane * 16);
+                shs[q] = *reinterpret_cast<const f32x4*>(reinterpret_cast<const char*>(a.sh_ws) + (size_t)tile * 4096 + q * 1024 + ln() * 16);
         }
         u32x4_t xah[KS], xal[KS], xbh[KS], xbl[KS];
         f32x16 denc[2];
@@ -313,6 +340,7 @@
         for (int t = 0; t < 2; ++t)
 #pragma unroll
             for (int e = 0; e < 16; ++e) denc[t][e] = 0.f;
+        char* dy_sig = dy_of(D);
 #pragma unroll
         for (int s = 0; s < KS; ++s) {
             const f32x4 wa = *reinterpret_cast<const f32x4*>(w2_h + 16 * s), wb = *reinterpret_cast<const f32x4*>(w2_h + 16 * s + 8);
@@ -327,22 +355,22 @@
                 xah[s][d] = mcn16_pkmul(wh, bits);
                 xal[s][d] = mcn16_pkmul(wl, bits);
             }
-            mcn16_ws_store(xah[s], reinterpret_cast<u32x4_t*>(dy_lane + (size_t)D * a.slot_bytes + s * 1024));
-            if (!HI) mcn16_ws_store(xal[s], reinterpret_cast<u32x4_t*>(dy_lane + (size_t)D * a.slot_bytes + (KS + s) * 1024));
+            mcn16_ws_store(xah[s], reinterpret_cast<u32x4_t*>(dy_sig + s * 1024));
+            if (!HI) mcn16_ws_store(xal[s], reinterpret_cast<u32x4_t*>(dy_sig + (KS + s) * 1024));
         }
         if (D >= 2) mask_issue(mask_lane, D - 2, buf_of(D - 2));
         unsigned mpend[MW];
-        if (!MASK_DMA && D >= 2) mask_read(mask_lane, mpend, 0, D - 2);
-        mcnx3_bwd_seg<W, KS, NT, 0, PPW, HI>(ring, smem, lane, xah, xal, xbh, xbl, mk_s, denc, nullptr);
+        if (!MASK_DMA && D >= 2) { if (ALT) mask_at(mpend, D - 2); else mask_read(mask_lane, mpend, 0, D - 2); }
+        mcnx3_bwd_seg<W, KS, NT, 0, PPW, HI, PF>(ring, smem, lane, xah, xal, xbh, xbl, mk_s, denc, nullptr);
         if (MASK_DMA) mask_read(mask_lane, mk_c, 1, D + 1);
         {
             u32x4_t dih[KS], dil[KS];
             dih[0] = dshh[0]; dih[1] = dshh[1]; dil[0] = dshl[0]; dil[1] = dshl[1];
-            mcnx3_bwd_seg<W, 2, NT, 1, PPW, HI>(ring, smem, lane, dih, dil, xah, xal, mk_c, denc, dy_lane + (size_t)(D + 1) * a.slot_bytes);
+            mcnx3_bwd_seg<W, 2, NT, 1, PPW, HI, PF>(ring, smem, lane, dih, dil, xah, xal, mk_c, denc, dy_of(D + 1));
         }
         if (D >= 3) mask_issue(mask_lane, D - 3, buf_of(D - 3));
         if (MASK_DMA) mask_read(mask_lane, mk_t, 2, D - 1);
-        mcnx3_bwd_seg<W, KS, NT, 2, PPW, HI>(ring, smem, lane, xah, xal, xbh, xbl, mk_t, denc, dy_lane + (size_t)(D - 1) * a.slot_bytes);
+        mcnx3_bwd_seg<W, KS, NT, 2, PPW, HI, PF>(ring, smem, lane, xah, xal, xbh, xbl, mk_t, denc, dy_of(D - 1));
         auto trunk_masks = [&](int l) {
             if (MASK_DMA) {
                 if (l >= 3) mask_issue(mask_lane, l - 3, buf_of(l - 3));
@@ -350,9 +378,9 @@
             } else {
 #pragma unroll
                 for (int i = 0; i < MW; ++i) mk_t[i] = mpend[i];
-                if (l >= 2) mask_read(mask_lane, mpend, 0, l - 2);
-            }
-            if (l == 1 && pass_n * ROWS < total) {
+                if (l >= 2) { if (ALT) mask_at(mpend, l - 2); else mask_read(mask_lane, mpend, 0, l - 2); }
+            }
+            if (!ALT && l == 1 && pass_n * ROWS < total) {
                 const unsigned* mln = mask_lane_of(pass_n);
                 mask_issue(mln, D, 0); mask_issue(mln, D + 1, 1); mask_issue(mln, D - 1, 2);
                 if (!MASK_DMA) { mask_read(mln, mk0_s, 0, D); mask_read(mln, mk0_c, 1, D + 1); mask_read(mln, mk0_t, 2, D - 1); }
@@ -365,7 +393,7 @@
                 const int2 rj = *reinterpret_cast<const int2*>(smem + SM::oIdx + wave * 256 + m * 8);
                 rn = rj.x; jn = rj.y;
             } else {
-                const long long gn = row_of(pass_n);
+                const long long gn = row_of(pass_n, m);
                 rn = (int)(gn / a.S); jn = (int)(gn - (long long)rn * a.S);
             }
             gather_dma(rn, jn);
@@ -374,13 +402,13 @@
         for (int l = D - 1; l >= 1; l -= 2) {
             if (PREFB && l == 1) next_rows();
             trunk_masks(l);
-            if (l == skip) mcnx3_bwd_seg<W, KS, 2, 3, PPW, HI>(ring, smem, lane, xbh, xbl, xah, xal, mk_t, denc, nullptr);
-            mcnx3_bwd_seg<W, KS, NT, 1, PPW, HI>(ring, smem, lane, xbh, xbl, xah, xal, mk_t, denc, dy_lane + (size_t)(l - 1) * a.slot_bytes);
+            if (l == skip) mcnx3_bwd_seg<W, KS, 2, 3, PPW, HI, PF>(ring, smem, lane, xbh, xbl, xah, xal, mk_t, denc, nullptr);
+            mcnx3_bwd_seg<W, KS, NT, 1, PPW, HI, PF>(ring, smem, lane, xbh, xbl, xah, xal, mk_t, denc, dy_of(l - 1));
             if (l - 1 >= 1) {
                 if (PREFB && l - 1 == 1) next_rows();
                 trunk_masks(l - 1);
-                if (l - 1 == skip) mcnx3_bwd_seg<W, KS, 2, 3, PPW, HI>(ring, smem, lane, xah, xal, xbh, xbl, mk_t, denc, nullptr);
-                mcnx3_bwd_seg<W, KS, NT, 1, PPW, HI>(ring, smem, lane, xah, xal, xbh, xbl, mk_t, denc, dy_lane + (size_t)(l - 2) * a.slot_bytes);
+                if (l - 1 == skip) mcnx3_bwd_seg<W, KS, 2, 3, PPW, HI, PF>(ring, smem, lane, xah, xal, xbh, xbl, mk_t, denc, nullptr);
+                mcnx3_bwd_seg<W, KS, NT, 1, PPW, HI, PF>(ring, smem, lane, xah, xal, xbh, xbl, mk_t, denc, dy_of(l - 2));
             } else {
 #pragma unroll
                 for (int s = 0; s < KS; ++s) { xbh[s] = xah[s]; xbl[s] = xal[s]; }
@@ -392,27 +420,28 @@
         }
         if (!PREFB) {
             int rn, jn;
+            const int m_n = ALT ? ln() & 31 : m;
             if (a.idx) {
-                const int2 rj = *reinterpret_cast<const int2*>(smem + SM::oIdx + wave * 256 + m * 8);
+                const int2 rj = *reinterpret_cast<const int2*>(smem + SM::oIdx + wave * 256 + m_n * 8);
                 rn = rj.x; jn = rj.y;
             } else {
-                const long long gn = row_of(pass_n);
+                const long long gn = row_of(pass_n, m_n);
                 rn = (int)(gn / a.S); jn = (int)(gn - (long long)rn * a.S);
             }
             nxt = gather(rn, jn);
         }
-        if (!PREFB && want_rays) {
+        if (!SHS_EARLY && want_rays) {
 #pragma unroll
             for (int q = 0; q < 4; ++q)
-                shs[q] = *reinterpret_cast<const f32x4*>(reinterpret_cast<const char*>(a.sh_ws) + (size_t)tile * 4096 + q * 1024 + lane * 16);
-        }
-        mcnx3_bwd_seg<W, KS, 2, 3, PPW, HI>(ring, smem, lane, xbh, xbl, xah, xal, mk_t, denc, nullptr);
+                shs[q] = *reinterpret_cast<const f32x4*>(reinterpret_cast<const char*>(a.sh_ws) + (size_t)tile * 4096 + q * 1024 + ln() * 16);
+        }
+        mcnx3_bwd_seg<W, KS, 2, 3, PPW, HI, PF>(ring, smem, lane, xbh, xbl, xah, xal, mk_t, denc, nullptr);
         auto settle = [&]() {
             if (PREFB && D >= 2) return;
             asm volatile("s_waitcnt vmcnt(0)" ::: "memory");
             asm volatile("" : "+v"(nxt.ray), "+v"(nxt.zg), "+v"(nxt.jit), "+v"(nxt.o), "+v"(nxt.go));
             asm volatile("" : "+v"(nxt.dx), "+v"(nxt.dy), "+v"(nxt.dz), "+v"(nxt.ox), "+v"(nxt.oy), "+v"(nxt.oz));
-            if (!MASK_DMA) {
+            if (!MASK_DMA && !ALT) {
 #pragma unroll
                 for (int i = 0; i < MW; ++i) asm volatile("" : "+v"(mk0_s[i]), "+v"(mk0_c[i]), "+v"(mk0_t[i]));
             }
@@ -478,7 +507,7 @@
                 if (m >= off) head |= hup;
             }
             const int rnext = __shfl_down(rkey, 1, 32);
-            if (h == 0 && valid && (m == 31 || rnext != rkey)) {
+            if (h == 0 && valid && !twin && (m == 31 || rnext != rkey)) {
 #pragma unroll
                 for (int c = 0; c < 3; ++c) {
                     if (a.d_rays_o) atomicAdd(a.d_rays_o + ray * 3 + c, red[c]);
@@ -492,10 +521,28 @@
     asm volatile("s_waitcnt vmcnt(0)" ::: "memory");
 }
 
+template <int W, bool HI>
+__global__ __launch_bounds__(64 * mcnx3_waves(W), mcnx3_waves(W) / 4) void mlp_x3_bwd_kernel(Mcn16BwdArgs a) {
+    mlp_x3_bwd_body<W, HI, mcnx3_waves(W)>(a);
+}
+template <int W, bool HI>
+__global__ __launch_bounds__(64 * mcnx3_alt_waves(W), mcnx3_alt_waves(W) / 4) void mlp_x3_bwd_kernel_alt(Mcn16BwdArgs a) {
+    mlp_x3_bwd_body<W, HI, mcnx3_alt_waves(W)>(a);
+}
+
 hipError_t mcnx3_launch_bwd(const Mcn16BwdArgs& a, hipStream_t st) {
     return mcn_for_width(a.lay.width, [&](auto w) {
-        constexpr int W = decltype(w)::value, WAVES = mcnx3_waves(W);
-        void (*kern)(Mcn16BwdArgs) = mcn16_hi_planes_only(a.dtype) ? mlp_x3_bwd_kernel<W, true> : mlp_x3_bwd_kernel<W, false>;
+        constexpr int W = decltype(w)::value;
+        const bool hi = mcn16_hi_planes_only(a.dtype);
+        if constexpr (mcnx3_has_alt_waves(W)) {
+            constexpr int WAVES = mcnx3_alt_waves(W);
+            if (mcnx3_w128_waves(MCNX3_CHAIN_BWD) == WAVES) {
+                void (*kern)(Mcn16BwdArgs) = hi ? mlp_x3_bwd_kernel_alt<W, true> : mlp_x3_bwd_kernel_alt<W, false>;
+                return mcn_launch(kern, mcn_persistent_grid(mcn_passes(mcn_max_rows(a), 32 * WAVES)), 64 * WAVES, BwdX3Smem<W, WAVES>::total, st, a);
+            }
+        }
+        constexpr int WAVES = mcnx3_waves(W);
+        void (*kern)(Mcn16BwdArgs) = hi ? mlp_x3_bwd_kernel<W, true> : mlp_x3_bwd_kernel<W, false>;
         return mcn_launch(kern, mcn_persistent_grid(mcn_passes(mcn_max_rows(a), 32 * WAVES)), 64 * WAVES, BwdX3Smem<W>::total, st, a);
     });
 }
diff --git a/mc_nerf_amd/csrc/mlp_x3_fwd.hip b/mc_nerf_amd/csrc/mlp_x3_fwd.hip
--- a/mc_nerf_amd/csrc/mlp_x3_fwd.hip
+++ b/mc_nerf_amd/csrc/mlp_x3_fwd.hip
@@ -1,17 +1,19 @@
 #include "mcnerf_x3.h"
 #include "mcnerf_launch.h"
-
-template <int W>
+#include "mcnerf_x3_waves.h"
+
+template <int W, int WV = mcnx3_waves(W)>
 struct FwdX3Smem {
     static constexpr int oBias = MCN16_RING * MCN16_SLAB * 1024;
     static constexpr int oW2 = oBias + (MCN_MAXD + 2) * W * 4;
     static constexpr int oBc2 = oW2 + W * 4;
     static constexpr int oIdx = oBc2 + 32 * 4;
-    static constexpr int oIn = oIdx + mcnx3_waves(W) * 256;
-    static constexpr int total = oIn + mcnx3_waves(W) * 8 * 256;
+    static constexpr int oIn = oIdx + WV * 256;
+    static constexpr int oKeep = oIn + WV * 8 * 256;
+    static constexpr int total = oKeep + (WV != mcnx3_waves(W) ? WV * 4 * 256 : 0);
 };
 
-template <int W, int SV, int KENC, int KHID, int EPI, int PPW>
+template <int W, int SV, int KENC, int KHID, int EPI, int PPW, int PF = MCNX3_PF>
 __device__ __forceinline__ void mcnx3_layer(Mcn16Ring& ring, char* smem, int lane,
                                             const u32x4_t (&ench)[MCN16_ENCKS], const u32x4_t (&encl)[MCN16_ENCKS],
                                             const u32x4_t (&inh)[W / 16], const u32x4_t (&inl)[W / 16],
@@ -38,7 +40,7 @@
     unsigned mw[MW];
 #pragma unroll
     for (int i = 0; i < MW; ++i) mw[i] = 0u;
-    u32x4_t afh[MCNX3_PF], afl[MCNX3_PF];
+    u32x4_t afh[PF], afl[PF];
     f32x16 acc[2];
     unsigned mb = 0u;
     float v0 = 0.f, v1 = 0.f;
@@ -82,7 +84,7 @@
     };
     cur.cur = ring.next_off;
 #pragma unroll
-    for (int i = 0; i < MCNX3_PF; ++i)
+    for (int i = 0; i < PF; ++i)
         if (i < F) {
             afh[i] = *reinterpret_cast<const u32x4_t*>(smem + ring.next_off + i * 2048 + lane * 16);
             afl[i] = *reinterpret_cast<const u32x4_t*>(smem + ring.next_off + i * 2048 + 1024 + lane * 16);
@@ -93,12 +95,12 @@
 #pragma unroll
         for (int s = 0; s < KTOT; ++s) {
             const int f = t * KTOT + s;
-            mcnx3_before_mfma_spread<F, PPW>(ring, cur, f);
-            const u32x4_t a_h = afh[f % MCNX3_PF], a_l = afl[f % MCNX3_PF];
-            if (f + MCNX3_PF < F) {
-                const unsigned o = mcnx3_frag_off(ring, cur, f, f + MCNX3_PF) + lane * 16;
-                afh[f % MCNX3_PF] = *reinterpret_cast<const u32x4_t*>(smem + o);
-                afl[f % MCNX3_PF] = *reinterpret_cast<const u32x4_t*>(smem + o + 1024);
+            mcnx3_before_mfma_spread<F, PPW, PF>(ring, cur, f);
+            const u32x4_t a_h = afh[f % PF], a_l = afl[f % PF];
+            if (f + PF < F) {
+                const unsigned o = mcnx3_frag_off(ring, cur, f, f + PF) + lane * 16;
+                afh[f % PF] = *reinterpret_cast<const u32x4_t*>(smem + o);
+                afl[f % PF] = *reinterpret_cast<const u32x4_t*>(smem + o + 1024);
             }
             const u32x4_t b_h = s < KENC ? ench[s < KENC ? s : 0] : inh[s >= KENC ? s - KENC : 0];
             const u32x4_t b_l = s < KENC ? encl[s < KENC ? s : 0] : inl[s >= KENC ? s - KENC : 0];
@@ -113,14 +115,14 @@
                         item(acc[(t - 1) & 1], t - 1, 8 * IPW + (gap - SBASE) / SSTR);
                 }
                 if (gap == BIAS_G && t + 1 < NT) bias_init(acc[(t + 1) & 1], t + 1);
-                mcnx3_gap_dma<F, PPW>(ring, 3 * f + g);
+                mcnx3_gap_dma<F, PPW, PF>(ring, 3 * f + g);
                 __builtin_amdgcn_sched_barrier(0);
                 acc[t & 1] = mcnx3_mfma(g == 0 ? a_l : a_h, g == 1 ? b_l : b_h, acc[t & 1]);
                 __builtin_amdgcn_sched_barrier(0);
             }
         }
     }
-    mcnx3_layer_end<F, PPW>(ring);
+    mcnx3_layer_end<F, PPW, PF>(ring);
 #pragma unroll
     for (int i = 0; i < NIT; ++i) item(acc[(NT - 1) & 1], NT - 1, i);
     if (SAVE) {
@@ -130,12 +132,12 @@
 }
 
 
-template <int W, int SV>
-__global__ __launch_bounds__(64 * mcnx3_waves(W), mcnx3_waves(W) / 4) void mlp_x3_fwd_kernel(Mcn16FwdArgs a) {
-    using SM = FwdX3Smem<W>;
+template <int W, int SV, int WV>
+__device__ __forceinline__ void mlp_x3_fwd_body(const Mcn16FwdArgs& a) {
+    using SM = FwdX3Smem<W, WV>;
     constexpr bool SAVE = SV != 0, HI = SV == 2;
     constexpr int PL = HI ? 1 : 2;
-    constexpr int WAVES = mcnx3_waves(W), ROWS = 32 * WAVES, PPW = 16 / WAVES;
+    constexpr int WAVES = WV, ROWS = 32 * WAVES, PPW = 16 / WAVES;
     constexpr int KS = W / 16, MW = W >= 64 ? W / 64 : 1;
     constexpr float SXW = MCNX3_SX * MCNX3_SW;
     extern __shared__ __attribute__((aligned(16))) char smem[];
@@ -165,7 +167,9 @@
     for (int f = 0; f < MCN_NFREQ; ++f) bw[f] = a.barf_w[f];
     __syncthreads();
 
-    constexpr bool PREF = WAVES == 4;
+    constexpr bool ALT = WV != mcnx3_waves(W);
+    constexpr bool PREF = WAVES == 4 || ALT;
+    constexpr int PF = ALT ? 1 : MCNX3_PF;
     constexpr int SLABS_FULL = (W / 32) * (W / 16) / MCNX3_SLABF, SLABS_L0 = ((W / 32) * MCN16_ENCKS + MCNX3_SLABF - 1) / MCNX3_SLABF;
     constexpr int SLABS_SH2 = (W / 16 + MCNX3_SLABF - 1) / MCNX3_SLABF;
     constexpr int N_IDX = PPW * (SLABS_L0 + SLABS_FULL - 1) < 63 ? PPW * (SLABS_L0 + SLABS_FULL - 1) : 63;
@@ -173,8 +177,13 @@
     const unsigned idx_lds = (unsigned)reinterpret_cast<size_t>((mcn16_lds_ptr_t)smem) + SM::oIdx + wave * 256;
     const unsigned in_lds = (unsigned)reinterpret_cast<size_t>((mcn16_lds_ptr_t)smem) + SM::oIn + wave * (8 * 256);
     const float* in_rd = reinterpret_cast<const float*>(smem + SM::oIn + wave * (8 * 256)) + lane;
-    auto row_of = [&](long long pass_) -> long long {
-        const long long g_ = (pass_ * WAVES + wave) * 32 + m;
+    const long long live_tiles = (total + 127) / 128 * 4;
+    auto tile_of = [&](long long pass_) -> long long {
+        const long long t_ = pass_ * WAVES + wave;
+        return ALT && t_ >= live_tiles ? t_ - 4 : t_;
+    };
+    auto row_of = [&](long long pass_, int m_) -> long long {
+        const long long g_ = tile_of(pass_) * 32 + m_;
         return g_ < total ? g_ : total - 1;
     };
     auto gather_dma = [&](int ray_, int j_) {
@@ -188,7 +197,7 @@
     };
     int ray_n = 0, j_n = 0;
     {
-        const long long gc0 = row_of(blockIdx.x);
+        const long long gc0 = row_of(blockIdx.x, m);
         if (a.idx) { const int2 rj = a.idx[gc0]; ray_n = rj.x; j_n = rj.y; }
         else { ray_n = (int)(gc0 / a.S); j_n = (int)(gc0 - (long long)ray_n * a.S); }
         if (PREF) {
@@ -203,8 +212,15 @@
     const float* bias_h = sbias + 4 * h;
     const float* w2_h = sw2 + 4 * h;
 
+    const int lane0 = lane, m0 = m, h0 = h;
+    const float *in_rd0 = in_rd, *bias_h0 = bias_h, *w2_h0 = w2_h;
     for (long long pass = blockIdx.x; pass * ROWS < total; pass += gridDim.x) {
-        const long long tile = pass * WAVES + wave;
+        const int lane = ALT ? mcnx3_opaque(lane0) : lane0, m = ALT ? lane & 31 : m0, h = ALT ? lane >> 5 : h0;
+        const float* in_rd = ALT ? reinterpret_cast<const float*>(smem + SM::oIn + wave * (8 * 256)) + lane : in_rd0;
+        const float* bias_h = ALT ? sbias + 4 * h : bias_h0;
+        const float* w2_h = ALT ? sw2 + 4 * h : w2_h0;
+        auto ln = [&]() { return ALT ? mcnx3_opaque(lane0) : lane; };
+        const long long tile = tile_of(pass);
         const long long g = tile * 32 + m;
         const bool valid = g < total;
         const long long gc = valid ? g : total - 1;
@@ -231,10 +247,15 @@
         p[1] = __fadd_rn(oy, __fmul_rn(dy, zv));
         p[2] = __fadd_rn(oz, __fmul_rn(dz, zv));
         if (PREF && a.idx) {
-            const long long gn = (pass_n * WAVES + wave) * 32 + (lane >> 1);
-            mcn16_dma4(reinterpret_cast<const int*>(a.idx) + 2 * (gn < total ? gn : total - 1) + (lane & 1), idx_lds);
-        }
-        const int addr = ray * a.S + j;
+            const int lane_i = ln();
+            const long long gn = tile_of(pass_n) * 32 + (lane_i >> 1);
+            mcn16_dma4(reinterpret_cast<const int*>(a.idx) + 2 * (gn < total ? gn : total - 1) + (lane_i & 1), idx_lds);
+        }
+        int addr = ray * a.S + j;
+        if (ALT) {
+            float* keep = reinterpret_cast<float*>(smem + SM::oKeep + wave * (4 * 256)) + ln();
+            keep[0] = dx; keep[64] = dy; keep[128] = dz; keep[192] = __int_as_float(addr);
+        }
         u32x4_t ench[MCN16_ENCKS], encl[MCN16_ENCKS];
         {
             float E[64];
@@ -249,10 +270,20 @@
                     ench[s][d] = wh; encl[s][d] = wl;
                 }
         }
-        char* act_lane = SAVE ? reinterpret_cast<char*>(a.act_ws) + (size_t)tile * (PL * KS) * 1024 + lane * 16 : nullptr;
-        unsigned* mask_lane = SAVE ? a.mask_ws + ((size_t)tile * 64 + lane) * MW : nullptr;
+        char* act_lane = SAVE && !ALT ? reinterpret_cast<char*>(a.act_ws) + (size_t)tile * (PL * KS) * 1024 + lane * 16 : nullptr;
+        unsigned* mask_lane = SAVE && !ALT ? a.mask_ws + ((size_t)tile * 64 + lane) * MW : nullptr;
+        auto act_of = [&](int l) -> char* {
+            if (!SAVE) return nullptr;
+            if (ALT) return reinterpret_cast<char*>(a.act_ws) + ((size_t)tile * (PL * KS) * 1024 + (size_t)l * a.slot_bytes) + ln() * 16;
+            return act_lane + (size_t)l * a.slot_bytes;
+        };
+        auto mask_of = [&](int l) -> unsigned* {
+            if (!SAVE) return nullptr;
+            if (ALT) return a.mask_ws + ((size_t)tile * 64 * MW + (size_t)l * a.mask_slot_words) + ln() * MW;
+            return mask_lane + (size_t)l * a.mask_slot_words;
+        };
         if (SAVE) {
-            char* e = reinterpret_cast<char*>(a.enc_ws) + (size_t)tile * (PL * MCN16_ENCKS) * 1024 + lane * 16;
+            char* e = reinterpret_cast<char*>(a.enc_ws) + (size_t)tile * (PL * MCN16_ENCKS) * 1024 + ln() * 16;
 #pragma unroll
             for (int s = 0; s < MCN16_ENCKS; ++s) {
                 mcn16_ws_store(ench[s], reinterpret_cast<u32x4_t*>(e + s * 1024));
@@ -262,37 +293,38 @@
 
         u32x4_t xah[KS], xal[KS], xbh[KS], xbl[KS];
         float dot = 0.f;
-        mcnx3_layer<W, SV, MCN16_ENCKS, 0, 0, PPW>(ring, smem, lane, ench, encl, xah, xal, xbh, xbl, bias_h, nullptr, dot, act_lane, mask_lane);
+        mcnx3_layer<W, SV, MCN16_ENCKS, 0, 0, PPW, PF>(ring, smem, lane, ench, encl, xah, xal, xbh, xbl, bias_h, nullptr, dot, act_of(0), mask_of(0));
         for (int l = 1; l < D; l += 2) {
-            char* sl = SAVE ? act_lane + (size_t)l * a.slot_bytes : nullptr;
-            unsigned* ml = SAVE ? mask_lane + (size_t)l * a.mask_slot_words : nullptr;
-            if (l == skip) mcnx3_layer<W, SV, MCN16_ENCKS, KS, 0, PPW>(ring, smem, lane, ench, encl, xbh, xbl, xah, xal, bias_h + l * W, nullptr, dot, sl, ml);
-            else mcnx3_layer<W, SV, 0, KS, 0, PPW>(ring, smem, lane, ench, encl, xbh, xbl, xah, xal, bias_h + l * W, nullptr, dot, sl, ml);
+            char* sl = act_of(l);
+            unsigned* ml = mask_of(l);
+            if (l == skip) mcnx3_layer<W, SV, MCN16_ENCKS, KS, 0, PPW, PF>(ring, smem, lane, ench, encl, xbh, xbl, xah, xal, bias_h + l * W, nullptr, dot, sl, ml);
+            else mcnx3_layer<W, SV, 0, KS, 0, PPW, PF>(ring, smem, lane, ench, encl, xbh, xbl, xah, xal, bias_h + l * W, nullptr, dot, sl, ml);
             if (l + 1 < D) {
-                sl = SAVE ? act_lane + (size_t)(l + 1) * a.slot_bytes : nullptr;
-                ml = SAVE ? mask_lane + (size_t)(l + 1) * a.mask_slot_words : nullptr;
-                if (l + 1 == skip) mcnx3_layer<W, SV, MCN16_ENCKS, KS, 0, PPW>(ring, smem, lane, ench, encl, xah, xal, xbh, xbl, bias_h + (l + 1) * W, nullptr, dot, sl, ml);
-                else mcnx3_layer<W, SV, 0, KS, 0, PPW>(ring, smem, lane, ench, encl, xah, xal, xbh, xbl, bias_h + (l + 1) * W, nullptr, dot, sl, ml);
+                sl = act_of(l + 1);
+                ml = mask_of(l + 1);
+                if (l + 1 == skip) mcnx3_layer<W, SV, MCN16_ENCKS, KS, 0, PPW, PF>(ring, smem, lane, ench, encl, xah, xal, xbh, xbl, bias_h + (l + 1) * W, nullptr, dot, sl, ml);
+                else mcnx3_layer<W, SV, 0, KS, 0, PPW, PF>(ring, smem, lane, ench, encl, xah, xal, xbh, xbl, bias_h + (l + 1) * W, nullptr, dot, sl, ml);
             } else {
 #pragma unroll
                 for (int s = 0; s < KS; ++s) { xbh[s] = xah[s]; xbl[s] = xal[s]; }
             }
         }
-        mcnx3_layer<W, SV, 0, KS, 1, PPW>(ring, smem, lane, ench, encl, xbh, xbl, xah, xal, bias_h + D * W, w2_h, dot,
-                                            SAVE ? act_lane + (size_t)D * a.slot_bytes : nullptr, SAVE ? mask_lane + (size_t)D * a.mask_slot_words : nullptr);
+        mcnx3_layer<W, SV, 0, KS, 1, PPW, PF>(ring, smem, lane, ench, encl, xbh, xbl, xah, xal, bias_h + D * W, w2_h, dot,
+                                            act_of(D), mask_of(D));
         if (PREF) {
             asm volatile("s_waitcnt vmcnt(%0)" ::"n"(N_IDX) : "memory");
+            const int m_n = ALT ? ln() & 31 : m;
             if (a.idx) {
-                const int2 rj = *reinterpret_cast<const int2*>(smem + SM::oIdx + wave * 256 + m * 8);
+                const int2 rj = *reinterpret_cast<const int2*>(smem + SM::oIdx + wave * 256 + m_n * 8);
                 ray_n = rj.x; j_n = rj.y;
             } else {
-                const long long gn = row_of(pass_n);
+                const long long gn = row_of(pass_n, m_n);
                 ray_n = (int)(gn / a.S); j_n = (int)(gn - (long long)ray_n * a.S);
             }
             gather_dma(ray_n, j_n);
         }
-        mcnx3_layer<W, SV, 0, KS, 0, PPW>(ring, smem, lane, ench, encl, xbh, xbl, xah, xal, bias_h + (D + 1) * W, nullptr, dot,
-                                            SAVE ? act_lane + (size_t)(D + 1) * a.slot_bytes : nullptr, SAVE ? mask_lane + (size_t)(D + 1) * a.mask_slot_words : nullptr);
+        mcnx3_layer<W, SV, 0, KS, 0, PPW, PF>(ring, smem, lane, ench, encl, xbh, xbl, xah, xal, bias_h + (D + 1) * W, nullptr, dot,
+                                            act_of(D + 1), mask_of(D + 1));
         f32x16 acc;
 #pragma unroll
         for (int q = 0; q < 4; ++q) {
@@ -314,10 +346,17 @@
 #pragma unroll
         for (int e = 0; e < 16; ++e) acc[e] *= 1.0f / SXW;
         if (SAVE) {
-            char* e = reinterpret_cast<char*>(a.sh_ws) + (size_t)tile * 4096 + lane * 16;
+            char* e = reinterpret_cast<char*>(a.sh_ws) + (size_t)tile * 4096 + ln() * 16;
 #pragma unroll
             for (int q = 0; q < 4; ++q)
                 mcn16_ws_store(f32x4{acc[4 * q], acc[4 * q + 1], acc[4 * q + 2], acc[4 * q + 3]}, reinterpret_cast<f32x4*>(e + q * 1024));
+        }
+        const int lane_e = ln();
+        const int h_e = ALT ? lane_e >> 5 : h;
+        const bool valid_e = ALT ? tile * 32 + (lane_e & 31) < total : valid;
+        if (ALT) {
+            const float* k = reinterpret_cast<const float*>(smem + SM::oKeep + wave * (4 * 256)) + lane_e;
+            dx = k[0]; dy = k[64]; dz = k[128]; addr = __float_as_int(k[192]);
         }
         float bas[9];
         mcn_sh_basis(dx, dy, dz, bas);
@@ -326,33 +365,51 @@
         for (int r = 0; r < 16; ++r) {
             const int n0 = 8 * (r >> 2) + (r & 3), n1 = n0 + 4;
             const float b0 = n0 < MCN_NSH ? bas[n0 % 9] : 0.f, b1 = n1 < MCN_NSH ? bas[n1 % 9] : 0.f;
-            const float contrib = acc[r] * (h ? b1 : b0);
+            const float contrib = acc[r] * (h_e ? b1 : b0);
             const int c0 = n0 / 9, c1 = n1 / 9;
 #pragma unroll
             for (int c = 0; c < 3; ++c) {
                 const bool in0 = n0 < MCN_NSH && c0 == c, in1 = n1 < MCN_NSH && c1 == c;
                 if (in0 && in1) pre[c] += contrib;
-                else if (in0) pre[c] += h ? 0.f : contrib;
-                else if (in1) pre[c] += h ? contrib : 0.f;
-            }
-        }
-        const float sigma = (dot + __shfl_xor(dot, 32)) * (1.0f / MCNX3_SX) + bs2;
+                else if (in0) pre[c] += h_e ? 0.f : contrib;
+                else if (in1) pre[c] += h_e ? contrib : 0.f;
+            }
+        }
+        const float sigma = (dot + (ALT ? mcnx3_swap32(dot, lane_e) : __shfl_xor(dot, 32))) * (1.0f / MCNX3_SX) + bs2;
         f32x4 o;
         o[0] = sigma;
 #pragma unroll
         for (int c = 0; c < 3; ++c) {
-            const float pc = pre[c] + __shfl_xor(pre[c], 32);
+            const float pc = pre[c] + (ALT ? mcnx3_swap32(pre[c], lane_e) : __shfl_xor(pre[c], 32));
             o[1 + c] = 1.0f / (1.0f + expf(-pc));
         }
-        if (valid && h == 0) *reinterpret_cast<f32x4*>(a.out + (size_t)addr * 4) = o;
+        if (valid_e && h_e == 0) *reinterpret_cast<f32x4*>(a.out + (size_t)addr * 4) = o;
     }
     asm volatile("s_waitcnt vmcnt(0)" ::: "memory");
 }
 
+template <int W, int SV>
+__global__ __launch_bounds__(64 * mcnx3_waves(W), mcnx3_waves(W) / 4) void mlp_x3_fwd_kernel(Mcn16FwdArgs a) {
+    mlp_x3_fwd_body<W, SV, mcnx3_waves(W)>(a);
+}
+template <int W, int SV>
+__global__ __launch_bounds__(64 * mcnx3_alt_waves(W), mcnx3_alt_waves(W) / 4) void mlp_x3_fwd_kernel_alt(Mcn16FwdArgs a) {
+    mlp_x3_fwd_body<W, SV, mcnx3_alt_waves(W)>(a);
+}
+
 hipError_t mcnx3_launch_fwd(const Mcn16FwdArgs& a, hipStream_t st) {
     return mcn_for_width(a.lay.width, [&](auto w) {
-        constexpr int W = decltype(w)::value, WAVES = mcnx3_waves(W);
-        void (*kern)(Mcn16FwdArgs) = !a.act_ws ? mlp_x3_fwd_kernel<W, 0> : mcn16_hi_planes_only(a.dtype) ? mlp_x3_fwd_kernel<W, 2> : mlp_x3_fwd_kernel<W, 1>;
+        constexpr int W = decltype(w)::value;
+        const int sv = !a.act_ws ? 0 : mcn16_hi_planes_only(a.dtype) ? 2 : 1;
+        if constexpr (mcnx3_has_alt_waves(W)) {
+            constexpr int WAVES = mcnx3_alt_waves(W);
+            if (sv != 1 && mcnx3_w128_waves(sv ? MCNX3_CHAIN_FWD_SAVE : MCNX3_CHAIN_FWD_NOSAVE) == WAVES) {
+                void (*kern)(Mcn16FwdArgs) = sv == 0 ? mlp_x3_fwd_kernel_alt<W, 0> : mlp_x3_fwd_kernel_alt<W, 2>;
+                return mcn_launch(kern, mcn_persistent_grid(mcn_passes(mcn_max_rows(a), 32 * WAVES)), 64 * WAVES, FwdX3Smem<W, WAVES>::total, st, a);
+            }
+        }
+        constexpr int WAVES = mcnx3_waves(W);
+        void (*kern)(Mcn16FwdArgs) = sv == 0 ? mlp_x3_fwd_kernel<W, 0> : sv == 2 ? mlp_x3_fwd_kernel<W, 2> : mlp_x3_fwd_kernel<W, 1>;
         return mcn_launch(kern, mcn_persistent_grid(mcn_passes(mcn_max_rows(a), 32 * WAVES)), 64 * WAVES, FwdX3Smem<W>::total, st, a);
     });
 }
```

Measured after the change: 1.103 million rays/s, median of 6. No clear change (+1.0%).
